# zypher-game/uzkge

Hardware: AMD Instinct MI355X
Metric: bn254_g1_msm_points_per_sec (higher is better)
Workload: dtype u256 (254-bit modular integers: 8 x u32 Montgomery limbs in HBM, 9 x 29-bit limbs in the two hot loops); 1 GPU; BN254 G1 MSM, 2^24 random points + uniform scalars per GPU, bases resident in HBM; points_per_gpu=16777216, total_points=16777216

## Files before the change

uzkge_amd/csrc/api.cpp:

```cpp
#include <algorithm>
#include <atomic>
#include <cstdarg>
#include <cstdlib>
#include <cstring>
#include <exception>
#include <new>

#include "anemoi29.hpp"
#include "ctx.hpp"
#include "fq12_29.hpp"
#include "g2_29.hpp"
#include "host_ec64.hpp"
#include "host_math.hpp"
#include "shufflecs_dev.hpp"
#include "matchcs_dev.hpp"

namespace uzk {

static thread_local char g_err[512] = "";

void set_error(const char* fmt, ...) {
    va_list ap;
    va_start(ap, fmt);
    vsnprintf(g_err, sizeof g_err, fmt, ap);
// ... 154 lines not shown
        device = c.want_device >= 0 ? c.want_device : s.device;
        UZK_TRY(device_cus_locked(s, device, &c.num_cus));
    }
    UZK_HIP(hipSetDevice(device));
    if (!c.ready) {
        UZK_HIP(hipStreamCreateWithFlags(&c.stream, hipStreamNonBlocking));
        c.device = device;
        c.ready = true;
    }
    return UZK_OK;
}

void devices_synchronize() {
    Shared& s = shared();
    std::vector<int> devs;
    {
        std::lock_guard<std::mutex> lk(s.mu);
        for (auto& kv : s.num_cus) devs.push_back(kv.first);
    }
    for (int d : devs) { (void)hipSetDevice(d); (void)hipDeviceSynchronize(); }
}

static void ctx_release(Ctx& c) {
    if (!c.ready) return;
    (void)hipSetDevice(c.device);
    (void)hipStreamSynchronize(c.stream);
    ntt_free_plans(c);
    g1ntt_free(c);
    srscheck_free(c);
    g2_free(c);
    g16_free(c);
    c.verify_ws.release();
    c.g16v_ws.release();
    c.ed_ws.release();
    c.shuffle_ws.release();
    c.match_ws.release();
    c.ed_gen.release();
    c.ed_gen_ready = false;
    c.pairing_ws.release();
    msm_free(c);
    poly_free(c);
    c.ntt_scratch[0].release(); c.ntt_scratch[1].release(); c.ntt_io.release(); c.msm_scalars.release();
    if (c.msm_tail_host) { (void)hipHostFree(c.msm_tail_host); c.msm_tail_host = nullptr; c.msm_tail_cap = 0; }
    for (auto& pe : c.prof_pending) { (void)hipEventDestroy(pe.e0); (void)hipEventDestroy(pe.e1); }
    c.prof_pending.clear();
    for (auto e : c.event_pool) (void)hipEventDestroy(e);
    c.event_pool.clear();
    (void)hipStreamDestroy(c.stream);
    c.stream = nullptr;
    c.cur_stream = nullptr;
    c.ready = false;
    c.device = -1;
}

static const Fp* as_fp(const uint64_t* p) { return reinterpret_cast<const Fp*>(p); }

static void copy_tuning(const Ctx& from, Ctx& to);
int ctx_init_internal(Ctx& c, int device) {
    c.want_device = device;
    {
        std::lock_guard<std::mutex> lk(default_ctx().mu);
        copy_tuning(default_ctx(), c);
    }
    CtxScope scope(&c);
    std::lock_guard<std::mutex> lk(c.mu);
    return require_ready();
}
void ctx_release_internal(Ctx& c) {
    std::lock_guard<std::mutex> lk(c.mu);
    ctx_release(c);
}

}

using namespace uzk;

#define API_LOCK std::lock_guard<std::mutex> _lk(ctx_mutex())

extern "C" {

#ifndef UZK_SRC_HASH
#define UZK_SRC_HASH "unstamped"
#endif
const char* uzk_version(void) { return "uzkge-amd 0.3 (gfx950) src:" UZK_SRC_HASH; }
const char* uzk_last_error(void) { return g_err; }

int uzk_device_count(void) try {
    int n = 0;
    if (hipGetDeviceCount(&n) != hipSuccess) return 0;
    return n;
} catch (...) { return uzk::on_exception("uzk_device_count"); }

int uzk_init(int device) try {
    API_LOCK;
    Shared& s = shared();
    {
        std::lock_guard<std::mutex> lk(s.mu);
        if (s.bound && s.device != device) {
            set_error("uzk_init(%d): already bound to device %d (one process per GPU)", device, s.device);
            return UZK_ERR_PARAMETER;
        }
        if (!s.bound) {
            int n = 0;
            if (hipGetDeviceCount(&n) != hipSuccess || n <= 0) {
                set_error("no HIP device visible: the MI355X backend has no CPU fallback");
                return UZK_ERR_DEVICE;
            }
            if (device < 0 || device >= n) {
                set_error("uzk_init(%d): %d device(s) visible", device, n);
                return UZK_ERR_PARAMETER;
            }
            UZK_TRY(bind_device_locked(s, device));
        }
    }
    return require_ready();
} catch (...) { return uzk::on_exception("uzk_init"); }

int uzk_shutdown(void) try {
    Shared& s = shared();
    coalesce_release_all();
    sharded_release_all();
    prover_release_all();
    vf_release_all();
    g2_release_all();
    g16_release_all();
    g16v_release_all();
    remark_release_all();
    std::lock_guard<std::mutex> lk(s.mu);
    if (!s.bound) return UZK_OK;
    ctx_release(default_ctx());
    for (auto& kv : s.contexts) { ctx_release(*kv.second); delete kv.second; }
    s.contexts.clear();
    s.epoch.fetch_add(1, std::memory_order_acq_rel);
    t_handle = 0;
    t_cached = nullptr;
    for (auto& kv : s.srs) {
        (void)hipSetDevice(kv.second.device);
        if (kv.second.owned && kv.second.d_points) (void)hipFree(kv.second.d_points);
        if (kv.second.d_table) (void)hipFree(kv.second.d_table);
    }
    s.srs.clear();
    s.num_cus.clear();
    s.bound = false;
    s.device = -1;
    return UZK_OK;
} catch (...) { return uzk::on_exception("uzk_shutdown"); }

namespace uzk {
static void copy_tuning(const Ctx& from, Ctx& to) {
    to.msm_window_bits = from.msm_window_bits;
    to.tune_no_precompute = from.tune_no_precompute; to.tune_ntt_tile = from.tune_ntt_tile; to.tune_ntt_two_pass = from.tune_ntt_two_pass; to.tune_small = from.tune_small;
    to.tune_chunk_log = from.tune_chunk_log; to.tune_verify_transcript = from.tune_verify_transcript; to.tune_stream_log = from.tune_stream_log; to.tune_stream_min_log = from.tune_stream_min_log;
    to.tune_seg_sort = from.tune_seg_sort; to.tune_arith29 = from.tune_arith29;
    to.tune_msm_taper = from.tune_msm_taper;
}
}
int uzk_ctx_create(uint64_t* ctx_out) try {
    if (!ctx_out) { set_error("uzk_ctx_create: null pointer"); return UZK_ERR_PARAMETER; }
    Ctx* c = new Ctx();
    {
        API_LOCK;
        int rc = require_ready();
        if (rc != UZK_OK) { delete c; return rc; }
        copy_tuning(ctx(), *c);
    }
    Shared& s = shared();
    std::lock_guard<std::mutex> lk(s.mu);
    const uint64_t h = s.next_ctx++;
    s.contexts[h] = c;
    *ctx_out = h;
    return UZK_OK;
} catch (...) { return uzk::on_exception("uzk_ctx_create"); }
int uzk_ctx_create_on(int device, uint64_t* ctx_out) try {
    if (!ctx_out) { set_error("uzk_ctx_create_on: null pointer"); return UZK_ERR_PARAMETER; }
    int n = 0;
    if (hipGetDeviceCount(&n) != hipSuccess || n <= 0) { set_error("no HIP device visible: the MI355X backend has no CPU fallback"); return UZK_ERR_DEVICE; }
    if (device < 0 || device >= n) { set_error("uzk_ctx_create_on(%d): %d device(s) visible", device, n); return UZK_ERR_PARAMETER; }
    Ctx* c = new Ctx();
    {
        API_LOCK;
        copy_tuning(ctx(), *c);
    }
    c->want_device = device;
    Shared& s = shared();
    std::lock_guard<std::mutex> lk(s.mu);
    const uint64_t h = s.next_ctx++;
    s.contexts[h] = c;
    *ctx_out = h;
    return UZK_OK;
} catch (...) { return uzk::on_exception("uzk_ctx_create_on"); }
int uzk_ctx_device(uint64_t handle, int* device_out) try {
    if (!device_out) { set_error("uzk_ctx_device: null pointer"); return UZK_ERR_PARAMETER; }
    Shared& s = shared();
    std::lock_guard<std::mutex> lk(s.mu);
    Ctx* c = nullptr;
    if (handle == 0) c = &default_ctx();
    else {
        auto it = s.contexts.find(handle);
        if (it == s.contexts.end()) { set_error("uzk_ctx_device: unknown context %llu", (unsigned long long)handle); return UZK_ERR_PARAMETER; }
        c = it->second;
    }
    *device_out = c->ready ? c->device : (c->want_device >= 0 ? c->want_device : (s.bound ? s.device : g_last_device));
    return UZK_OK;
} catch (...) { return uzk::on_exception("uzk_ctx_device"); }
int uzk_ctx_set_current(uint64_t handle) try {
    if (handle == 0) { t_handle = 0; t_cached = nullptr; return UZK_OK; }
    Shared& s = shared();
    std::lock_guard<std::mutex> lk(s.mu);
    auto it = s.contexts.find(handle);
    if (it == s.contexts.end()) { set_error("uzk_ctx_set_current: unknown context %llu", (unsigned long long)handle); return UZK_ERR_PARAMETER; }
    t_handle = handle;
    t_cached = it->second;
    t_epoch = s.epoch.load(std::memory_order_acquire);
    return UZK_OK;
} catch (...) { return uzk::on_exception("uzk_ctx_set_current"); }
int uzk_ctx_destroy(uint64_t handle) try {
    Shared& s = shared();
    Ctx* c = nullptr;
    {
        std::lock_guard<std::mutex> lk(s.mu);
        auto it = s.contexts.find(handle);
        if (it == s.contexts.end()) { set_error("uzk_ctx_destroy: unknown context %llu", (unsigned long long)handle); return UZK_ERR_PARAMETER; }
        c = it->second;
        s.contexts.erase(it);
        s.epoch.fetch_add(1, std::memory_order_acq_rel);
    }
    if (t_handle == handle) { t_handle = 0; t_cached = nullptr; }
    { std::lock_guard<std::mutex> lk(c->mu); ctx_release(*c); }
    delete c;
    return UZK_OK;
} catch (...) { return uzk::on_exception("uzk_ctx_destroy"); }

int uzk_ctx_current(uint64_t* ctx_out) try {
    if (!ctx_out) { set_error("uzk_ctx_current: null pointer"); return UZK_ERR_PARAMETER; }
    (void)ctx();
    *ctx_out = t_handle;
    return UZK_OK;
} catch (...) { return uzk::on_exception("uzk_ctx_current"); }
int uzk_ctx_wait(uint64_t other) try {
    Ctx* cur = &ctx();
    Ctx* oth = nullptr;
    if (other == 0) oth = &default_ctx();
    else {
        Shared& s = shared();
        std::lock_guard<std::mutex> lk(s.mu);
        auto it = s.contexts.find(other);
        if (it == s.contexts.end()) { set_error("uzk_ctx_wait: unknown context %llu", (unsigned long long)other); return UZK_ERR_PARAMETER; }
        oth = it->second;
    }
    if (oth == cur) return UZK_OK;
    std::unique_lock<std::mutex> l1(cur->mu, std::defer_lock), l2(oth->mu, std::defer_lock);
    std::lock(l1, l2);
    UZK_TRY(require_ready());
    if (!oth->ready) return UZK_OK;
    hipEvent_t ev = oth->get_event();
    struct Return { Ctx* c; hipEvent_t e; ~Return() { c->event_pool.push_back(e); } } back{oth, ev};
    UZK_HIP(hipEventRecord(ev, oth->stream));
    UZK_HIP(hipStreamWaitEvent(cur->stream, ev, 0));
    return UZK_OK;
} catch (...) { return uzk::on_exception("uzk_ctx_wait"); }

int uzk_dev_alloc(size_t bytes, void** d_out) try {
    API_LOCK;
    if (!d_out) { set_error("uzk_dev_alloc: null pointer"); return UZK_ERR_PARAMETER; }
    *d_out = nullptr;
    UZK_TRY(require_ready());
    if (bytes == 0) return UZK_OK;
    hipError_t e = hipMalloc(d_out, bytes);
    if (e != hipSuccess) {
        (void)hipGetLastError();
        *d_out = nullptr;
        set_error("uzk_dev_alloc(%zu): %s", bytes, hipGetErrorString(e));
        return UZK_ERR_DEVICE;
    }
    return UZK_OK;
} catch (...) { return uzk::on_exception("uzk_dev_alloc"); }
int uzk_dev_free(void* d_ptr) try {
    API_LOCK;
    if (!d_ptr) return UZK_OK;
    UZK_TRY(require_ready());
    UZK_HIP(hipStreamSynchronize(ctx().stream));
    UZK_HIP(hipFree(d_ptr));
    return UZK_OK;
} catch (...) { return uzk::on_exception("uzk_dev_free"); }
int uzk_host_alloc(size_t bytes, void** h_out) try {
    API_LOCK;
    if (!h_out) { set_error("uzk_host_alloc: null pointer"); return UZK_ERR_PARAMETER; }
    *h_out = nullptr;
    UZK_TRY(require_ready());
    if (bytes == 0) return UZK_OK;
    hipError_t e = hipHostMalloc(h_out, bytes, hipHostMallocDefault);
    if (e != hipSuccess) { (void)hipGetLastError(); *h_out = nullptr; set_error("uzk_host_alloc(%zu): %s", bytes, hipGetErrorString(e)); return UZK_ERR_DEVICE; }
    Shared& s = shared();
    std::lock_guard<std::mutex> lk(s.mu);
    s.pinned[*h_out] = bytes;
    return UZK_OK;
} catch (...) { return uzk::on_exception("uzk_host_alloc"); }
int uzk_host_free(void* h_ptr) try {
    API_LOCK;
    if (!h_ptr) return UZK_OK;
    UZK_TRY(require_ready());
    Shared& s = shared();
    size_t bytes = 0;
    {
        std::lock_guard<std::mutex> lk(s.mu);
        auto it = s.pinned.find(h_ptr);
        if (it == s.pinned.end()) { set_error("uzk_host_free: %p is not a block of uzk_host_alloc", h_ptr); return UZK_ERR_PARAMETER; }
// ... 1352 lines not shown
    API_LOCK;
    if (n > 0 && (!a || !b || !out)) { set_error("uzk_test_g2_kat: null pointer"); return UZK_ERR_PARAMETER; }
    if (op < 0 || (op > 5 && op < 10) || op > 14) { set_error("uzk_test_g2_kat: bad op"); return UZK_ERR_PARAMETER; }
    UZK_TRY(require_ready());
    return g2_op_device(ctx(), op, a, b, out, n);
} catch (...) { return uzk::on_exception("uzk_test_g2_kat"); }

int uzk_test_l29_kat(int field, int op, uint32_t param, const uint32_t* in, uint32_t* out, size_t n) try {
    API_LOCK;
    if (n > 0 && (!in || !out)) { set_error("uzk_test_l29_kat: null pointer"); return UZK_ERR_PARAMETER; }
    if (field < 0 || field > 1 || op < 0 || op > 22) { set_error("uzk_test_l29_kat: bad field/op"); return UZK_ERR_PARAMETER; }
    if (op == 20 && param > 5) { set_error("uzk_test_l29_kat: sub_off takes offsets 0 .. 5"); return UZK_ERR_PARAMETER; }
    if (op == 21 && !l29_sig_runnable(field, param)) { set_error("uzk_test_l29_kat: not a sub / to_wire / canon signature of this field"); return UZK_ERR_PARAMETER; }
    UZK_TRY(require_ready());
    return l29_op_device(ctx(), field, op, param, in, out, n);
} catch (...) { return uzk::on_exception("uzk_test_l29_kat"); }
int uzk_test_p29_kat(int op, const uint32_t* in, uint32_t* out, size_t n) try {
    API_LOCK;
    if (n > 0 && (!in || !out)) { set_error("uzk_test_p29_kat: null pointer"); return UZK_ERR_PARAMETER; }
    if (op < 0 || op > 3) { set_error("uzk_test_p29_kat: bad op"); return UZK_ERR_PARAMETER; }
    UZK_TRY(require_ready());
    return p29_op_device(ctx(), op, in, out, n);
} catch (...) { return uzk::on_exception("uzk_test_p29_kat"); }
int uzk_test_g2_raw_kat(int op, const uint32_t* in, uint32_t* out, size_t n) try {
    API_LOCK;
    if (n > 0 && (!in || !out)) { set_error("uzk_test_g2_raw_kat: null pointer"); return UZK_ERR_PARAMETER; }
    if (op < 0 || op > 4) { set_error("uzk_test_g2_raw_kat: bad op"); return UZK_ERR_PARAMETER; }
    UZK_TRY(require_ready());
    return g2_raw_op_device(ctx(), op, in, out, n);
} catch (...) { return uzk::on_exception("uzk_test_g2_raw_kat"); }
int uzk_test_fq12_raw_kat(int op, const uint32_t* in, uint32_t* out, size_t n) try {
    API_LOCK;
    if (n > (1u << 20) || (n > 0 && (!in || !out))) { set_error("uzk_test_fq12_raw_kat: null pointer or more than 2^20 elements"); return UZK_ERR_PARAMETER; }
    if (op < 0 || op > 12) { set_error("uzk_test_fq12_raw_kat: bad op"); return UZK_ERR_PARAMETER; }
    UZK_TRY(require_ready());
    return pairing_raw_kat_device(ctx(), op, in, out, (uint32_t)n);
} catch (...) { return uzk::on_exception("uzk_test_fq12_raw_kat"); }
int uzk_test_miller_step_raw(int op, const uint32_t* in, uint32_t* out, size_t n) try {
    API_LOCK;
    if (n > (1u << 20) || (n > 0 && (!in || !out))) { set_error("uzk_test_miller_step_raw: null pointer or more than 2^20 records"); return UZK_ERR_PARAMETER; }
    if (op < 0 || op > 1) { set_error("uzk_test_miller_step_raw: bad op"); return UZK_ERR_PARAMETER; }
    UZK_TRY(require_ready());
    return pairing_raw_step_device(ctx(), op, in, out, (uint32_t)n);
} catch (...) { return uzk::on_exception("uzk_test_miller_step_raw"); }
int uzk_test_ed_raw_kat(int op, const uint32_t* in, uint32_t* out, size_t n) try {
    API_LOCK;
    if (n > 0 && (!in || !out)) { set_error("uzk_test_ed_raw_kat: null pointer"); return UZK_ERR_PARAMETER; }
    if (op < 0 || op > 6) { set_error("uzk_test_ed_raw_kat: bad op"); return UZK_ERR_PARAMETER; }
    UZK_TRY(require_ready());
    return ed_raw_op_device(ctx(), op, in, out, n);
} catch (...) { return uzk::on_exception("uzk_test_ed_raw_kat"); }
int uzk_test_lanes(int op, const void* const* d_polys, const uint64_t* lane_strides, uint32_t count, const uint32_t* lens, const uint32_t* pts,
                   const uint64_t* args, uint32_t lanes, uint64_t len, uint64_t* out, int* kernel) try {
    API_LOCK;
    if (op < 0 || op > 1 || count == 0 || lanes == 0 || !kernel) { set_error("uzk_test_lanes: bad op / count / lanes"); return UZK_ERR_PARAMETER; }
    if (!d_polys || !lane_strides || !lens || !args || !out || (op == 1 && !pts)) { set_error("uzk_test_lanes: null pointer"); return UZK_ERR_PARAMETER; }
    for (uint32_t k = 0; k < count; ++k)
        if (!d_polys[k] || (op == 1 && pts[k] > 1)) { set_error("uzk_test_lanes: null polynomial or point index > 1"); return UZK_ERR_PARAMETER; }
    UZK_TRY(require_ready());
    return lanes_test(ctx(), op, d_polys, lane_strides, count, lens, pts, as_fp(args), lanes, len, reinterpret_cast<Fp*>(out), kernel);
} catch (...) { return uzk::on_exception("uzk_test_lanes"); }
int uzk_test_ntt_in_len(const void* d_in, uint64_t in_stride, void* d_out, uint64_t out_stride, uint64_t n, uint32_t batch,
                        const uint64_t* coset_shift_mont, uint64_t in_len) try {
    API_LOCK;
    if (!domain_supported(n)) {
        set_error("no evaluation domain of size %llu (need 2^k, k <= %d, or 3 * 2^k, k <= %d)", (unsigned long long)n, UZK_NTT_MAX_LOG2, UZK_NTT_MAX_LOG2_MIXED);
        return UZK_ERR_FFT;
    }
    if (!d_in || !d_out) { set_error("uzk_test_ntt_in_len: null pointer"); return UZK_ERR_PARAMETER; }
    UZK_TRY(require_ready());
    Ctx& c = ctx();
    UZK_TRY(ntt_run(c, static_cast<const Fp*>(d_in), static_cast<Fp*>(d_out), n, false,
                    coset_shift_mont ? as_fp(coset_shift_mont) : nullptr, batch, in_stride, out_stride, in_len));
    UZK_HIP(hipStreamSynchronize(c.stream));
    return UZK_OK;
} catch (...) { return uzk::on_exception("uzk_test_ntt_in_len"); }

int uzk_profile_enable(int on) try {
    API_LOCK;
    UZK_TRY(require_ready());
    Ctx& c = ctx();
    UZK_TRY(c.prof_collect());
    c.prof_on = on != 0;
    return UZK_OK;
} catch (...) { return uzk::on_exception("uzk_profile_enable"); }
int uzk_profile_reset(void) try {
    API_LOCK;
    Ctx& c = ctx();
    if (c.ready) UZK_TRY(c.prof_collect());
    c.prof_totals.clear();
    return UZK_OK;
} catch (...) { return uzk::on_exception("uzk_profile_reset"); }
int uzk_profile_get(const char* name, double* total_ms, uint64_t* launches) try {
    API_LOCK;
    Ctx& c = ctx();
    if (!name) { set_error("uzk_profile_get: null name"); return UZK_ERR_PARAMETER; }
    if (c.ready) UZK_TRY(c.prof_collect());
    auto it = c.prof_totals.find(name);
    if (total_ms) *total_ms = (it == c.prof_totals.end()) ? 0.0 : it->second.first;
    if (launches) *launches = (it == c.prof_totals.end()) ? 0 : it->second.second;
    return UZK_OK;
} catch (...) { return uzk::on_exception("uzk_profile_get"); }
int uzk_profile_dump(char* buf, size_t cap) try {
    API_LOCK;
    Ctx& c = ctx();
    if (!buf || cap == 0) { set_error("uzk_profile_dump: null buffer"); return UZK_ERR_PARAMETER; }
    if (c.ready) UZK_TRY(c.prof_collect());
    size_t off = 0;
    buf[0] = 0;
    for (auto& kv : c.prof_totals) {
        int w = snprintf(buf + off, cap - off, "%s %llu %.6f\n", kv.first.c_str(),
                         (unsigned long long)kv.second.second, kv.second.first);
        if (w < 0 || (size_t)w >= cap - off) break;
        off += (size_t)w;
    }
    return UZK_OK;
} catch (...) { return uzk::on_exception("uzk_profile_dump"); }
int uzk_sync(void) try {
    API_LOCK;
    UZK_TRY(require_ready());
    UZK_HIP(hipStreamSynchronize(ctx().stream));
    return UZK_OK;
} catch (...) { return uzk::on_exception("uzk_sync"); }
void* uzk_stream(void) {
    API_LOCK;
    if (require_ready() != UZK_OK) return nullptr;
    return ctx().stream;
}
int uzk_msm_set_window_bits(int c) try {
    API_LOCK;
    if (c != 0 && (c < 4 || c > 22)) { set_error("window bits must be 0 (auto) or 4..22"); return UZK_ERR_PARAMETER; }
    ctx().msm_window_bits = c;
    return UZK_OK;
} catch (...) { return uzk::on_exception("uzk_msm_set_window_bits"); }

int uzk_msm_plan_info(size_t n, int* window_bits, int* windows) try {
    API_LOCK;
    if (!window_bits || !windows || n == 0) { set_error("uzk_msm_plan_info: bad arguments"); return UZK_ERR_PARAMETER; }
    msm_plan_info(ctx(), n, window_bits, windows);
    return UZK_OK;
} catch (...) { return uzk::on_exception("uzk_msm_plan_info"); }

int uzk_tune(const char* key, int value) try {
    API_LOCK;
    if (!key) { set_error("uzk_tune: null key"); return UZK_ERR_PARAMETER; }
    Ctx& c = ctx();
    if (!std::strcmp(key, "msm_no_precompute")) c.tune_no_precompute = value;
    else if (!std::strcmp(key, "msm_stream_log")) c.tune_stream_log = (value >= -1 && value <= 26) ? value : 0;
    else if (!std::strcmp(key, "msm_stream_min_log")) c.tune_stream_min_log = (value >= 4 && value <= 26) ? value : 22;
    else if (!std::strcmp(key, "msm_chunk_log")) c.tune_chunk_log = (value >= 8 && value <= 26) ? value : 26;
    else if (!std::strcmp(key, "msm_small")) c.tune_small = value ? 1 : 0;
    else if (!std::strcmp(key, "msm_seg_sort")) c.tune_seg_sort = value;
    else if (!std::strcmp(key, "msm_taper")) c.tune_msm_taper = (value >= 0 && value <= 2) ? value : 1;
    else if (!std::strcmp(key, "ntt_tile")) c.tune_ntt_tile = (value == 1024 || value == 2048) ? value : 0;
    else if (!std::strcmp(key, "ntt_two_pass")) c.tune_ntt_two_pass = value ? 1 : 0;
    else if (!std::strcmp(key, "arith29")) c.tune_arith29 = value & 7;
    else if (!std::strcmp(key, "verify_transcript")) c.tune_verify_transcript = (value == 1 || value == 2) ? value : 0;
    else { set_error("uzk_tune: unknown key %s", key); return UZK_ERR_PARAMETER; }
    return UZK_OK;
} catch (...) { return uzk::on_exception("uzk_tune"); }

}
```

uzkge_amd/csrc/ctx.hpp:

```cpp
#pragma once
#include <hip/hip_runtime.h>

#include <cstdint>
#include <cstdlib>
#include <cstdio>
#include <chrono>
#include <map>
#include <mutex>
#include <string>
#include <vector>

#include "../../include/uzkge_gpu.h"
#include "../../include/uzkge_gpu_test.h"
#include "ec.hpp"

namespace uzk {

void set_error(const char* fmt, ...);
int on_exception(const char* fn) noexcept;

#define UZK_HIP(expr)                                                                      \
    do {                                                                                   \
        hipError_t _e = (expr);                                                            \
        if (_e != hipSuccess) {                                                            \
            (void)hipGetLastError();  \
            ::uzk::set_error("%s failed: %s (%s:%d)", #expr, hipGetErrorString(_e), __FILE__, __LINE__); \
            return UZK_ERR_DEVICE;                                                         \
        }                                                                                  \
    } while (0)

#define UZK_TRY(expr)                  \
    do {                               \
        int _rc = (expr);              \
        if (_rc != UZK_OK) return _rc; \
    } while (0)

struct DevBuf {
    void* p = nullptr;
    size_t cap = 0;
    int reserve(size_t bytes);
    void release();
    template <class T> T* as() const { return reinterpret_cast<T*>(p); }
};

struct ArgArena {
    char* h = nullptr;
    char* d = nullptr;
    size_t cap = 0, used = 0, uploaded = 0;
    int init(size_t bytes);
    void release();
    void reset() { used = 0; uploaded = 0; }
    template <class T> T* push(size_t count, const T** dev) {
        const size_t at = (used + 15) & ~(size_t)15, bytes = count * sizeof(T);
        if (at + bytes > cap) { *dev = nullptr; return nullptr; }
        used = at + bytes;
        *dev = reinterpret_cast<const T*>(d + at);
        return reinterpret_cast<T*>(h + at);
    }
    int upload(hipStream_t s);
};

struct ProfEntry {
    std::string name;
    hipEvent_t e0, e1;
};

struct NttPlan;
struct MsmWork;

struct Ctx {
    std::mutex mu;
    bool ready = false;
    int want_device = -1;
    int device = -1;
    hipStream_t stream = nullptr;
    hipStream_t stream2 = nullptr;
    hipStream_t cur_stream = nullptr;
    int num_cus = 256;
    bool prof_on = false;
    std::vector<ProfEntry> prof_pending;
    std::vector<hipEvent_t> event_pool;
    std::map<std::string, std::pair<double, uint64_t>> prof_totals;
    std::map<uint64_t, NttPlan*> ntt_plans;
    DevBuf ntt_scratch[2];
    DevBuf ntt_io;
    MsmWork* msm = nullptr;
    DevBuf msm_scalars;
    Fp* msm_tail_host = nullptr;
    size_t msm_tail_cap = 0;
    int msm_window_bits = 0;
    int tune_no_precompute = 0;
    int tune_ntt_two_pass = 1;
    int tune_ntt_tile = 0;
    int tune_small = 1;
    int tune_chunk_log = 26;
    int tune_stream_log = 0;
    int tune_stream_min_log = 22;
    int tune_arith29 = default_arith29();
    static int default_arith29() {
        static const int v = [] { const char* e = std::getenv("UZK_ARITH29"); return e ? std::atoi(e) : 7; }();
        return v;
    }
    int tune_seg_sort = 1;
    int tune_msm_taper = 1;
    DevBuf poly_tmp, poly_tmp2, poly_io, zpoly_tmp, open_tmp, poly_args;
    DevBuf poly_cnt;
    uint32_t trim_flip = 0;
    void* poly_host = nullptr;
    size_t poly_host_cap = 0;
    DevBuf ntt_sub;
    struct PowCache { Fp key; bool valid = false; uint64_t stamp = 0; DevBuf buf; };
    PowCache pow_cache[8];
    uint64_t pow_stamp = 0;
    std::vector<void*> ntt_fused;
    std::map<uint64_t, void*> g1ntt_plans;
    DevBuf g1ntt_work, g1ntt_prefix, g1ntt_io;
    DevBuf verify_ws;
    DevBuf srs_records, srs_weights, srs_points;
    void* g2 = nullptr;
    void* g16 = nullptr;
    DevBuf g16v_ws;
    DevBuf pairing_ws;
    std::vector<uint8_t> pairing_status;
    DevBuf ed_ws;
    DevBuf ed_gen;
    bool ed_gen_ready = false;
    DevBuf shuffle_ws;
    DevBuf match_ws;
    int tune_verify_transcript = 0;
    struct Srs {
        Affine* d_points = nullptr;
        size_t n = 0;
        bool owned = false;
        int device = 0;
        Affine* d_table = nullptr;
        int pre_c = 0;
        uint32_t pre_W = 0;
    };

    hipEvent_t get_event();
    void prof_begin(const char* name);
    void prof_end();
    int prof_collect();
};

struct ScalarView {
    const Fp* main = nullptr;
    uint64_t stride = 0;
    uint32_t n_main = 0;
    const Fp* tail = nullptr;
    uint32_t tail_n = 0;
    uint32_t group = 0xffffffffu;
    uint64_t group_stride = 0;
    static ScalarView dense(const Fp* p, size_t n) { ScalarView v; v.main = p; v.stride = n; v.n_main = (uint32_t)n; return v; }
    __host__ __device__ const Fp& at(uint32_t b, uint32_t i) const {
        return i < n_main ? main[(uint64_t)(b / group) * group_stride + (uint64_t)(b % group) * stride + i]
                          : tail[(uint64_t)b * tail_n + (i - n_main)];
    }
};

Ctx& ctx();
std::mutex& ctx_mutex();
int require_ready();
struct CtxScope {
    Ctx* prev;
    explicit CtxScope(Ctx* c);
    ~CtxScope();
    CtxScope(const CtxScope&) = delete;
    CtxScope& operator=(const CtxScope&) = delete;
};
int ctx_init_internal(Ctx& c, int device);
void ctx_release_internal(Ctx& c);
void devices_synchronize();
void coalesce_release_all();
void sharded_release_all();
uint64_t srs_insert(const Ctx::Srs& e);
bool srs_lookup(uint64_t handle, Ctx::Srs* out);
bool srs_erase(uint64_t handle, Ctx::Srs* out);
bool is_pinned_block(const void* p, size_t bytes);
int msm_dispatch_view(const Ctx::Srs& s, size_t offset, const ScalarView& sv, size_t n, uint32_t batch, Jac* out);
void prover_release_all();

struct HostScope {
    Ctx& c;
    const char* name;
    std::chrono::steady_clock::time_point t0;
    HostScope(Ctx& c_, const char* n) : c(c_), name(n), t0(std::chrono::steady_clock::now()) {}
    ~HostScope() {
        if (!c.prof_on) return;
        const double ms = std::chrono::duration<double, std::milli>(std::chrono::steady_clock::now() - t0).count();
        auto& e = c.prof_totals[name];
        e.first += ms; e.second += 1;
    }
};

struct KernelScope {
    Ctx& c;
    KernelScope(Ctx& c_, const char* name) : c(c_) { if (c.prof_on) c.prof_begin(name); }
    ~KernelScope() { if (c.prof_on) c.prof_end(); }
};

#define UZK_LAUNCH(c, name, kernel, grid, block, lds, stream, ...)                        \
    do {                                                                                   \
        {                                                                                  \
            ::uzk::KernelScope _ks((c), (name));                                           \
            hipLaunchKernelGGL(kernel, grid, block, lds, stream, __VA_ARGS__);             \
        }                                                                                  \
        UZK_HIP(hipGetLastError());                                                        \
    } while (0)

struct DeviceGuard {
    int prev = -1;
    explicit DeviceGuard(int device) {
        (void)hipGetDevice(&prev);
        (void)hipSetDevice(device);
    }
    ~DeviceGuard() { if (prev >= 0) (void)hipSetDevice(prev); }
    DeviceGuard(const DeviceGuard&) = delete;
    DeviceGuard& operator=(const DeviceGuard&) = delete;
};

int ntt_run(Ctx& c, const Fp* d_in, Fp* d_out, uint64_t n, bool inverse, const Fp* coset_shift_host, uint32_t batch,
            uint64_t in_stride = 0, uint64_t out_stride = 0, uint64_t in_len = 0);
void ntt_free_plans(Ctx& c);
int g1ntt_run(Ctx& c, const Affine* d_in, Affine* d_out, uint64_t n, bool inverse);
void g1ntt_op_count(uint64_t n, bool inverse, uint64_t* dbl_out, uint64_t* add_out);
void g1ntt_free(Ctx& c);
int vf_key_check(const uzk_vk_desc* d);
int vf_key_create(Ctx& c, const uzk_vk_desc* d, uint64_t* out);
bool vf_key_known(uint64_t h, uint32_t* cs_size, uint32_t* n_pi, uint32_t* proof_bytes, int* device);
int vf_key_release(uint64_t h);
void vf_release_all();
int vf_key_set_public_key(Ctx& c, uint64_t h, const Affine* pk);
int vf_fold_run(Ctx& c, uint64_t h, const uint8_t* proofs, const Fp* pi, uint32_t m, const Fp* weights, Jac* left_out, Jac* right_out,
                uint8_t* status_out, Fp* challenges_out);
int vf_keccak_test(Ctx& c, const uint8_t* msgs, const uint64_t* offsets, uint32_t count, uint8_t* out);
int srs_curve_run(Ctx& c, const Affine* d_points, uint64_t count, uzk_srs_curve_report* out);
int srs_weights_run(Ctx& c, const uint8_t seed[32], uint64_t first, uint64_t count, Fp* d_out);
void srs_weights_host(const uint8_t seed[32], uint64_t first, uint64_t count, Fp* out);
void srscheck_free(Ctx& c);
struct G2Affine;
struct G2Jac;
int g2_register(Ctx& c, const G2Affine* points, size_t n, uint64_t* handle_out);
bool g2_lookup(uint64_t handle, const G2Affine** d_points, size_t* n, int* device);
bool g2_release(uint64_t handle);
void g2_release_all();
void g2_free(Ctx& c);
int g2_msm_run(Ctx& c, const G2Affine* d_points, const Fp* d_scalars, size_t n, uint32_t batch, G2Jac* out_host);
void g2_fold_host(const G2Jac* partials, size_t count, G2Jac* out);
void g2_to_affine_host(const G2Jac* p, G2Affine* out);
int g2_op_device(Ctx& c, int op, const uint64_t* a, const uint64_t* b, uint64_t* out, size_t n);
int g2_raw_op_device(Ctx& c, int op, const uint32_t* in, uint32_t* out, size_t n);
int g16_key_check(const uzk_g16_key_desc* d, uint64_t* domain_out);
int g16_key_create(Ctx& c, const uzk_g16_key_desc* d, uint64_t* out);
bool g16_key_known(uint64_t h, uint32_t* n_vars, uint32_t* n_inputs, uint32_t* n_constraints, uint64_t* domain, int* device);
bool g16_key_release(uint64_t h);
void g16_release_all();
// ... 124 lines not shown
```

uzkge_amd/csrc/msm.hip:

```cpp
#include <algorithm>
#include <cmath>
#include <mutex>
#include <functional>
#include <memory>
#include <condition_variable>
#include <atomic>
#include <cstring>
#include <thread>
#include <vector>

#include "ctx.hpp"
#include "ec29.hpp"
#include "ecquad.hpp"
#include "ecquad29.hpp"
#include "ec29l.hpp"
#include "host_ec64.hpp"
#include "host_math.hpp"
#include "msm_cut.hpp"

namespace uzk {

constexpr uint32_t kSeg = 16;
constexpr uint32_t kSignBit = 0x80000000u;
constexpr uint32_t kCombineFan = 32;
// ... 48 lines not shown
        uint32_t out;
        if (d > half) { out = ((1u << c) - d) | kSignBit; carry = 1; }
        else { out = d; carry = 0; }
        if (out & ~kSignBit) out ^= flip;
        if (w >= w0) dst[(size_t)(w - w0) * n] = out;
    }
}

__global__ __launch_bounds__(1024) void msm_digits_hist_kernel(ScalarView scalars, uint32_t* __restrict__ digits,
                                                               uint32_t n, int c, int W, uint32_t shift, uint32_t bins,
                                                               uint32_t* __restrict__ counts) {
    extern __shared__ uint32_t hist[];
    const uint32_t ch = blockIdx.x, nch = gridDim.x, b = blockIdx.y;
    const uint32_t cs = (n + nch - 1) / nch;
    const uint32_t lo = min(n, ch * cs), hi = min(n, lo + cs);
    for (uint32_t k = threadIdx.x; k < (uint32_t)W * bins; k += blockDim.x) hist[k] = 0;
    __syncthreads();
    const uint32_t mask = (1u << c) - 1, half = 1u << (c - 1), bmask = bins - 1;
    for (uint32_t i = lo + threadIdx.x; i < hi; i += blockDim.x) {
        Fp k = Fr::from_mont(scalars.at(b, i));
        const uint32_t flip = msm_fold_scalar_sign(k);
        uint32_t carry = 0;
        uint32_t* dst = digits + (size_t)b * W * n + i;
        for (int w = 0; w < W; ++w) {
            uint32_t d = (k.v[0] & mask) + carry;
#pragma unroll
            for (int j = 0; j < 7; ++j) k.v[j] = __funnelshift_r(k.v[j], k.v[j + 1], c);
            k.v[7] >>= c;
            uint32_t out;
            if (d > half) { out = ((1u << c) - d) | kSignBit; carry = 1; }
            else { out = d; carry = 0; }
            if (out & ~kSignBit) out ^= flip;
            dst[(size_t)w * n] = out;
            const uint32_t mag = out & ~kSignBit;
            if (mag) atomicAdd(&hist[(uint32_t)w * bins + (((mag - 1) >> shift) & bmask)], 1u);
        }
    }
    __syncthreads();
    for (uint32_t k = threadIdx.x; k < (uint32_t)W * bins; k += blockDim.x) {
        const uint32_t w = k / bins, bin = k % bins;
        counts[(((size_t)b * W + w) * nch + ch) * bins + bin] = hist[k];
    }
}

struct RadixArgs {
    const uint32_t* digits;
    const uint2* in_entries;
    const uint32_t* seg_start;
    const uint32_t* seg_len;
    uint32_t n;
    uint32_t remap_cnt;
    uint32_t remap_stride, remap_off;
    const uint32_t* item_off;
    uint32_t nseg, chunk;
    uint32_t shift, mask, bins;
    uint32_t* counts;
    uint32_t* prefix;
    uint32_t* bin_base;
    uint32_t* bin_count;
    uint2* out_entries;
    uint32_t* out_vals;
    uint32_t pk_in_bits, pk_out_bits;
    uint32_t seg_min_len;
};
__device__ __forceinline__ uint32_t pk_key(uint32_t e, uint32_t idx_bits) { return e >> (idx_bits + 1); }
__device__ __forceinline__ uint32_t pk_val(uint32_t e, uint32_t idx_bits) {
    return (e & ((1u << idx_bits) - 1)) | (((e >> idx_bits) & 1u) << 31);
}
__device__ __forceinline__ uint32_t pk_make(uint32_t key_low, uint32_t val, uint32_t idx_bits) {
    return (key_low << (idx_bits + 1)) | ((val >> 31) << idx_bits) | (val & ~kSignBit);
}

template <bool FROM_DIGITS>
__device__ __forceinline__ bool radix_work(const RadixArgs& a, uint32_t item, uint32_t& seg, size_t& cidx, uint32_t& base,
                                           uint32_t& lo, uint32_t& hi) {
    if constexpr (FROM_DIGITS) {
        const uint32_t ch = blockIdx.x, nch = gridDim.x;
        seg = blockIdx.y;
        cidx = ((size_t)seg * nch + ch) * a.bins;
        base = 0;
        const uint32_t cs = (a.n + nch - 1) / nch;
        lo = min(a.n, ch * cs);
        hi = min(a.n, lo + cs);
        return true;
    } else {
        if (item >= a.item_off[a.nseg]) return false;
        uint32_t l = 0, h = a.nseg;
        while (h - l > 1) {
            const uint32_t mid = (l + h) >> 1;
            if (a.item_off[mid] <= item) l = mid; else h = mid;
        }
        seg = l;
        cidx = (size_t)item * a.bins;
        base = a.seg_start[seg];
        const uint32_t len = a.seg_len[seg];
        lo = min(len, (item - a.item_off[seg]) * a.chunk);
        hi = min(len, lo + a.chunk);
        return true;
    }
}
template <bool FROM_DIGITS, bool PK_IN>
__device__ __forceinline__ bool radix_load(const RadixArgs& a, uint32_t seg, uint32_t base, uint32_t k, uint32_t& key,
                                           uint32_t& val) {
    if constexpr (FROM_DIGITS) {
        const uint32_t d = a.digits[(size_t)seg * a.n + k];
        const uint32_t mag = d & ~kSignBit;
        key = mag - 1;
        uint32_t idx = k;
        if (a.remap_cnt) idx = (k / a.remap_cnt) * a.remap_stride + a.remap_off + (k % a.remap_cnt);
        val = idx | (d & kSignBit);
        return mag != 0;
    } else if constexpr (PK_IN) {
        const uint32_t e = reinterpret_cast<const uint32_t*>(a.in_entries)[(size_t)base + k];
        key = pk_key(e, a.pk_in_bits);
        val = pk_val(e, a.pk_in_bits);
        return true;
    } else {
        const uint2 e = a.in_entries[(size_t)base + k];
        key = e.x;
        val = e.y;
        return true;
    }
}

template <bool FROM_DIGITS, bool PK_IN>
__global__ __launch_bounds__(1024) void msm_radix_hist_kernel(RadixArgs a) {
    __shared__ uint32_t cnt[512];
    for (uint32_t item = blockIdx.x;; item += gridDim.x) {
        uint32_t seg, base, lo, hi;
        size_t cidx;
        if (!radix_work<FROM_DIGITS>(a, item, seg, cidx, base, lo, hi)) return;
        for (uint32_t b = threadIdx.x; b < a.bins; b += blockDim.x) cnt[b] = 0;
        __syncthreads();
        for (uint32_t k = lo + threadIdx.x; k < hi; k += blockDim.x) {
            if constexpr (FROM_DIGITS) {
                const uint32_t mag = a.digits[(size_t)seg * a.n + k] & ~kSignBit;
                if (mag) atomicAdd(&cnt[((mag - 1) >> a.shift) & a.mask], 1u);
            } else if constexpr (PK_IN) {
                const uint32_t e = reinterpret_cast<const uint32_t*>(a.in_entries)[(size_t)base + k];
                atomicAdd(&cnt[(pk_key(e, a.pk_in_bits) >> a.shift) & a.mask], 1u);
            } else {
                atomicAdd(&cnt[(a.in_entries[(size_t)base + k].x >> a.shift) & a.mask], 1u);
            }
        }
        __syncthreads();
        uint32_t* dst = a.counts + cidx;
        for (uint32_t b = threadIdx.x; b < a.bins; b += blockDim.x) dst[b] = cnt[b];
        if constexpr (FROM_DIGITS) return;
        __syncthreads();
    }
}

__global__ __launch_bounds__(512) void msm_radix_scan_kernel(RadixArgs a, uint32_t nch, const uint32_t* __restrict__ out_start_of,
                                                             uint32_t out_stride) {
    __shared__ uint32_t wsum[8];
    const uint32_t seg = blockIdx.x, b = threadIdx.x, G = gridDim.y, g = blockIdx.y;
    if (a.seg_min_len && a.seg_len[seg] <= a.seg_min_len) return;
    uint32_t run = 0;
    if (b < a.bins) {
        size_t first = (size_t)seg * nch;
        uint32_t cnt = nch;
        if (a.item_off) { first = a.item_off[seg]; cnt = a.item_off[seg + 1] - a.item_off[seg]; }
        const uint32_t per = (cnt + G - 1) / G;
        const uint32_t c0 = min(cnt, g * per), c1 = min(cnt, c0 + per);
        const uint32_t* p0 = a.counts + first * a.bins + b;
        uint32_t r0 = 0, r1 = 0, r2 = 0, r3 = 0;
        uint32_t ch = 0;
        for (; ch + 4 <= c0; ch += 4) {
            r0 += p0[(size_t)ch * a.bins];
            r1 += p0[(size_t)(ch + 1) * a.bins];
            r2 += p0[(size_t)(ch + 2) * a.bins];
            r3 += p0[(size_t)(ch + 3) * a.bins];
        }
        for (; ch < c0; ++ch) r0 += p0[(size_t)ch * a.bins];
        run = r0 + r1 + r2 + r3;
        for (ch = c0; ch < c1; ++ch) {
            const size_t at = (first + ch) * a.bins + b;
            const uint32_t v = a.counts[at];
            a.prefix[at] = run;
            run += v;
        }
    }
    if (g + 1 != G) return;
    uint32_t incl = run;
    for (int o = 1; o < 64; o <<= 1) {
        const uint32_t t = __shfl_up((int)incl, o);
        if ((int)(b & 63) >= o) incl += t;
    }
    if ((b & 63) == 63) wsum[b >> 6] = incl;
    __syncthreads();
    uint32_t pre = 0;
    for (uint32_t w = 0; w < (b >> 6); ++w) pre += wsum[w];
    const uint32_t excl = pre + incl - run;
    if (b < a.bins) {
        const uint32_t start = out_start_of ? out_start_of[seg] : seg * out_stride;
        a.bin_base[(size_t)seg * a.bins + b] = start + excl;
        a.bin_count[(size_t)seg * a.bins + b] = run;
    }
}

__global__ __launch_bounds__(1024) void msm_radix_items_kernel(const uint32_t* __restrict__ seg_len, uint32_t nseg,
                                                               uint32_t chunk, uint32_t* __restrict__ item_off, uint32_t min_len) {
    __shared__ uint32_t part[1024];
    const uint32_t tid = threadIdx.x;
    const uint32_t per = (nseg + 1023) / 1024;
    const uint32_t lo = min(nseg, tid * per), hi = min(nseg, lo + per);
    uint32_t s = 0;
    auto items_of = [&](uint32_t k) { const uint32_t l = seg_len[k]; return l > min_len ? (l + chunk - 1) / chunk : 0u; };
    for (uint32_t k = lo; k < hi; ++k) s += items_of(k);
    part[tid] = s;
    __syncthreads();
    for (uint32_t off = 1; off < 1024; off <<= 1) {
        uint32_t v = (tid >= off) ? part[tid - off] : 0;
        __syncthreads();
        part[tid] += v;
        __syncthreads();
    }
    uint32_t run = part[tid] - s;
    for (uint32_t k = lo; k < hi; ++k) { item_off[k] = run; run += items_of(k); }
    if (tid == 1023) item_off[nseg] = part[1023];
}

template <int TB, int E, bool FROM_DIGITS, bool OUT_VAL, bool PK_IN>
__global__ __launch_bounds__(TB) void msm_radix_scatter_kernel(RadixArgs a) {
    constexpr int TILE = TB * E;
    __shared__ uint2 buf[TILE];
    __shared__ uint32_t tcnt[512], toff[512], gcur[512], wsum[16];
    const uint32_t tid = threadIdx.x;
    for (uint32_t item = blockIdx.x;; item += gridDim.x) {
    uint32_t seg, base, lo, hi;
    size_t cidx;
    if (!radix_work<FROM_DIGITS>(a, item, seg, cidx, base, lo, hi)) return;
    const uint32_t* coff = a.prefix + cidx;
    for (uint32_t b = tid; b < a.bins; b += TB) gcur[b] = a.bin_base[(size_t)seg * a.bins + b] + coff[b];
    for (uint32_t t0 = lo; t0 < hi; t0 += TILE) {
        for (uint32_t b = tid; b < a.bins; b += TB) tcnt[b] = 0;
        __syncthreads();
        uint32_t key[E], val[E], rank[E];
        bool ok[E];
#pragma unroll
        for (int e = 0; e < E; ++e) {
            const uint32_t k = t0 + tid + e * TB;
            ok[e] = (k < hi) && radix_load<FROM_DIGITS, PK_IN>(a, seg, base, k, key[e], val[e]);
            if (ok[e]) rank[e] = atomicAdd(&tcnt[(key[e] >> a.shift) & a.mask], 1u);
        }
        __syncthreads();
        {
            const uint32_t ngroups = (a.bins + 63) / 64, lane = tid & 63;
            for (uint32_t g = tid >> 6; g < ngroups; g += TB / 64) {
                const uint32_t b = g * 64 + lane;
                const uint32_t v = (b < a.bins) ? tcnt[b] : 0;
                uint32_t incl = v;
                for (int o = 1; o < 64; o <<= 1) {
                    const uint32_t t = __shfl_up((int)incl, o);
                    if ((int)lane >= o) incl += t;
                }
                if (b < a.bins) toff[b] = incl - v;
                if (lane == 63) wsum[g] = incl;
            }
            __syncthreads();
            for (uint32_t b = tid; b < a.bins; b += TB) {
                uint32_t pre = 0;
                for (uint32_t g = 0; g < (b >> 6); ++g) pre += wsum[g];
                toff[b] += pre;
            }
            __syncthreads();
        }
#pragma unroll
        for (int e = 0; e < E; ++e) {
            if (ok[e]) buf[toff[(key[e] >> a.shift) & a.mask] + rank[e]] = make_uint2(key[e], val[e]);
        }
        __syncthreads();
        const uint32_t last = a.bins - 1;
        const uint32_t total = toff[last] + tcnt[last];
        for (uint32_t k = tid; k < total; k += TB) {
            const uint2 en = buf[k];
            const uint32_t bin = (en.x >> a.shift) & a.mask;
            const uint32_t pos = gcur[bin] + (k - toff[bin]);
            if constexpr (OUT_VAL) a.out_vals[pos] = en.y;
            else if (a.pk_out_bits)
                reinterpret_cast<uint32_t*>(a.out_entries)[pos] = pk_make(en.x & ((1u << a.shift) - 1), en.y, a.pk_out_bits);
            else a.out_entries[pos] = en;
        }
        __syncthreads();
        for (uint32_t b = tid; b < a.bins; b += TB) gcur[b] += tcnt[b];
        __syncthreads();
    }
    if constexpr (FROM_DIGITS) return;
    }
}

template <int TB, int E, int BUFN>
__global__ __launch_bounds__(TB, TB >= 512 ? 4 : 2) void msm_radix_segment_kernel(RadixArgs a) {
    constexpr uint32_t CAP = (uint32_t)TB * E;
    constexpr int MAXBINS = 512;
    __shared__ uint32_t buf[BUFN];
    __shared__ uint32_t cnt[MAXBINS], off[MAXBINS + 1], cur[MAXBINS], wsum[8];
    const uint32_t seg = blockIdx.x, tid = threadIdx.x;
    const uint32_t len = a.seg_len[seg];
    if (len > CAP) return;
    const uint32_t start = a.seg_start[seg];
    const uint32_t bins = a.bins;
    for (uint32_t b = tid; b < bins; b += TB) cnt[b] = 0;
    __syncthreads();
    const uint32_t* __restrict__ in = reinterpret_cast<const uint32_t*>(a.in_entries) + start;
    uint32_t e[E];
    const int mine = tid < len ? (int)((len - tid + TB - 1) / TB) : 0;
#pragma unroll
    for (int i = 0; i < E; ++i) e[i] = i < mine ? in[tid + (uint32_t)i * TB] : 0u;
#pragma unroll
    for (int i = 0; i < E; ++i)
        if (i < mine) atomicAdd(&cnt[(pk_key(e[i], a.pk_in_bits) >> a.shift) & a.mask], 1u);
    __syncthreads();
    {
        const uint32_t ngroups = (bins + 63) / 64, lane = tid & 63;
        for (uint32_t g = tid >> 6; g < ngroups; g += TB / 64) {
            const uint32_t b = g * 64 + lane;
            const uint32_t v = (b < bins) ? cnt[b] : 0;
            uint32_t incl = v;
            for (int o = 1; o < 64; o <<= 1) {
                const uint32_t t = __shfl_up((int)incl, o);
                if ((int)lane >= o) incl += t;
            }
            if (b < bins) off[b] = incl - v;
            if (lane == 63) wsum[g] = incl;
        }
        __syncthreads();
        for (uint32_t b = tid; b < bins; b += TB) {
            uint32_t pre = 0;
            for (uint32_t g = 0; g < (b >> 6); ++g) pre += wsum[g];
            const uint32_t o = off[b] + pre;
            off[b] = o;
            cur[b] = o;
            a.bin_base[(size_t)seg * bins + b] = start + o;
            a.bin_count[(size_t)seg * bins + b] = cnt[b];
        }
        if (tid == 0) off[bins] = len;
        __syncthreads();
    }
    uint32_t* __restrict__ out = a.out_vals + start;
    uint32_t b_lo = 0;
    while (b_lo < bins) {
        const uint32_t base = off[b_lo];
        uint32_t l = b_lo, h = bins + 1;
        while (h - l > 1) {
            const uint32_t mid = (l + h) >> 1;
            if (off[mid] - base <= (uint32_t)BUFN) l = mid; else h = mid;
        }
        const bool direct = (l == b_lo);
        const uint32_t b_hi = direct ? b_lo + 1 : l;
#pragma unroll
        for (int i = 0; i < E; ++i) {
            asm volatile("" : "+v"(e[i]));
            const uint32_t bin = (pk_key(e[i], a.pk_in_bits) >> a.shift) & a.mask;
            if (i < mine && bin >= b_lo && bin < b_hi) {
                const uint32_t pos = atomicAdd(&cur[bin], 1u);
                const uint32_t val = pk_val(e[i], a.pk_in_bits);
                if (direct) out[pos] = val; else buf[pos - base] = val;
            }
        }
        __syncthreads();
        if (!direct) {
            const uint32_t total = off[b_hi] - base;
            for (uint32_t k = tid; k < total; k += TB) out[base + k] = buf[k];
            __syncthreads();
        }
        b_lo = b_hi;
    }
}

template <int TB, int E, int BUFN>
__global__ __launch_bounds__(TB, 4) void msm_radix_chunk_kernel(RadixArgs a) {
    constexpr int MAXBINS = 512;
// ... 265 lines not shown
                                                               uint32_t* __restrict__ cursor, TaskDesc* __restrict__ desc) {
    const uint32_t n_big = *big_count, lane = threadIdx.x;
    for (uint32_t i = blockIdx.x; i < n_big; i += gridDim.x) {
        const BigBucket e = big[i];
        const uint32_t q = e.total / e.T, r = e.total - q * e.T;
        uint32_t p_hi = 0, p_lo = 0;
        if (lane == 0) {
            if (r) p_hi = atomicAdd(&cursor[min(q + 1, kLenBins - 1)], r);
            p_lo = atomicAdd(&cursor[min(q, kLenBins - 1)], e.T - r);
        }
        p_hi = (uint32_t)__shfl((int)p_hi, 0);
        p_lo = (uint32_t)__shfl((int)p_lo, 0);
        for (uint32_t j = lane; j < e.T; j += 64) {
            TaskDesc d;
            d.start = e.start + j * q + min(j, r);
            d.cnt = q + (j < r ? 1u : 0u);
            d.task = e.tid0 + j;
            d.pad = 0;
            desc[j < r ? p_hi + j : p_lo + (j - r)] = d;
        }
    }
}

__device__ __forceinline__ XYZZ& task_dst(XYZZ* __restrict__ partials, XYZZ* __restrict__ direct, uint32_t task) {
    return (task & kSignBit) ? direct[task & ~kSignBit] : partials[task];
}
__global__ __launch_bounds__(256, 4) void msm_accumulate29_kernel(const Affine* __restrict__ points,
                                                                  const uint32_t* __restrict__ sorted,
                                                                  const TaskDesc* __restrict__ desc,
                                                                  const uint32_t* __restrict__ win_base,
                                                                  XYZZ* __restrict__ partials, uint32_t W,
                                                                  uint32_t* __restrict__ exc_count,
                                                                  uint32_t* __restrict__ exc_list, XYZZ* __restrict__ direct = nullptr) {
#if defined(__HIP_DEVICE_COMPILE__)
    const uint32_t slot = blockIdx.x * blockDim.x + threadIdx.x;
    if (slot >= win_base[W]) return;
    const TaskDesc d = desc[slot];
    const uint32_t cnt = d.cnt;
    const uint32_t* run = sorted + d.start;
    Acc29 acc = acc29_inf();
    uint32_t e = run[0];
    Affine p = load_point(points, e & ~kSignBit);
    for (uint32_t k = 0; k < cnt; ++k) {
        const Affine cur = p;
        const bool neg = (e & kSignBit) != 0;
        if (k + 1 < cnt) {
            e = run[k + 1];
            p = load_point(points, e & ~kSignBit);
        }
        if (!acc29_madd(acc, cur, neg)) {
            exc_list[atomicAdd(exc_count, 1u)] = slot;
            return;
        }
    }
    task_dst(partials, direct, d.task) = acc29_to_xyzz(acc);
#endif
}
__global__ __launch_bounds__(256) void msm_accumulate_exc_kernel(const Affine* __restrict__ points,
                                                                 const uint32_t* __restrict__ sorted,
                                                                 const TaskDesc* __restrict__ desc,
                                                                 XYZZ* __restrict__ partials,
                                                                 const uint32_t* __restrict__ exc_count,
                                                                 const uint32_t* __restrict__ exc_list, XYZZ* __restrict__ direct = nullptr) {
    const uint32_t total = *exc_count;
    for (uint32_t i = blockIdx.x * blockDim.x + threadIdx.x; i < total; i += gridDim.x * blockDim.x) {
        const TaskDesc d = desc[exc_list[i]];
        const uint32_t* run = sorted + d.start;
        XYZZ acc = xyzz_inf();
        for (uint32_t k = 0; k < d.cnt; ++k) {
            const uint32_t e = run[k];
            xyzz_madd(acc, load_point(points, e & ~kSignBit), (e & kSignBit) != 0);
        }
        task_dst(partials, direct, d.task) = acc;
    }
}

__device__ __forceinline__ XYZZ xyzz_shfl_down(const XYZZ& p, int delta) {
    XYZZ r;
    const uint32_t* s = reinterpret_cast<const uint32_t*>(&p);
    uint32_t* d = reinterpret_cast<uint32_t*>(&r);
#pragma unroll
    for (int k = 0; k < 32; ++k) d[k] = (uint32_t)__shfl_down((int)s[k], delta);
    return r;
}
template <int GS>
__device__ __forceinline__ XYZZ fold_partials29(const XYZZ* __restrict__ src, uint32_t cnt, uint32_t sub) {
    P29 acc = p29_inf();
    for (uint32_t k = sub; k < cnt; k += GS) { const P29 q = p29_load(src[k]); p29_add(acc, q); }
    for (int o = GS / 2; o > 0; o >>= 1) {
        P29 q;
        const uint32_t* sp = reinterpret_cast<const uint32_t*>(&acc);
        uint32_t* dp = reinterpret_cast<uint32_t*>(&q);
#pragma unroll
        for (int w = 0; w < 36; ++w) dp[w] = (uint32_t)__shfl_down((int)sp[w], o);
        if (sub + (uint32_t)o < (uint32_t)GS) p29_add(acc, q);
    }
    return sub == 0 ? p29_store(acc) : xyzz_inf();
}
template <int GS>
__device__ __forceinline__ XYZZ fold_partials(const XYZZ* __restrict__ src, uint32_t cnt, uint32_t sub) {
    XYZZ acc = xyzz_inf();
    for (uint32_t k = sub; k < cnt; k += GS) { XYZZ q = src[k]; xyzz_add(acc, q); }
    for (int o = GS / 2; o > 0; o >>= 1) {
        XYZZ q = xyzz_shfl_down(acc, o);
        if (sub + (uint32_t)o < (uint32_t)GS) xyzz_add(acc, q);
    }
    return acc;
}

struct BigFold { uint32_t src, cnt, dst, pad; };
template <int GS>
__global__ __launch_bounds__(256) void msm_combine_kernel(const XYZZ* __restrict__ in, const uint32_t* __restrict__ in_cnt,
                                                          const uint32_t* __restrict__ in_off,
                                                          const uint32_t* __restrict__ in_base,
                                                          const uint32_t* __restrict__ task_off,
                                                          const uint32_t* __restrict__ win_base, XYZZ* __restrict__ out,
                                                          uint32_t NB, uint32_t W, uint32_t G, uint32_t* __restrict__ big_count,
                                                          BigFold* __restrict__ big, uint32_t big_thresh, int arith29) {
    const uint32_t gt = blockIdx.x * blockDim.x + threadIdx.x;
    const uint32_t tid = gt / GS, sub = gt % GS;
    if (tid >= win_base[W]) return;
    uint32_t w, b, j;
    find_task(tid, win_base, W, task_off, NB, w, b, j);
    const uint32_t total = in_cnt[(size_t)w * NB + b];
    const uint32_t first = j * G;
    const uint32_t cnt = min(G, total - first);
    const uint32_t at = in_base[w] + in_off[(size_t)w * NB + b] + first;
    if (GS == 1 && big != nullptr && cnt > big_thresh) {
        BigFold e; e.src = at; e.cnt = cnt; e.dst = tid; e.pad = 0;
        big[atomicAdd(big_count, 1u)] = e;
        return;
    }
    XYZZ acc = arith29 ? fold_partials29<GS>(in + at, cnt, sub) : fold_partials<GS>(in + at, cnt, sub);
    if (sub == 0) out[tid] = acc;
}
__global__ __launch_bounds__(64) void msm_fold_big_kernel(const XYZZ* __restrict__ in, const uint32_t* __restrict__ big_count,
                                                          const BigFold* __restrict__ big, XYZZ* __restrict__ out, int accumulate) {
    const uint32_t total = *big_count, lane = threadIdx.x;
    for (uint32_t i = blockIdx.x; i < total; i += gridDim.x) {
        const BigFold e = big[i];
        XYZZ acc = xyzz_inf();
        for (uint32_t k = lane; k < e.cnt; k += 64) { XYZZ q = in[e.src + k]; xyzz_add(acc, q); }
        for (int o = 32; o > 0; o >>= 1) {
            XYZZ q = xyzz_shfl_down(acc, o);
            if (lane + (uint32_t)o < 64) xyzz_add(acc, q);
        }
        if (lane == 0) {
            if (accumulate) { XYZZ prev = out[e.dst]; xyzz_add(prev, acc); out[e.dst] = prev; }
            else out[e.dst] = acc;
        }
    }
}

template <int GS>
__global__ __launch_bounds__(256) void msm_finalize_kernel(const XYZZ* __restrict__ in, const uint32_t* __restrict__ in_cnt,
                                                           const uint32_t* __restrict__ in_off,
                                                           const uint32_t* __restrict__ in_base,
                                                           XYZZ* __restrict__ buckets, uint32_t NB, uint32_t W, int accumulate,
                                                           uint32_t* __restrict__ big_count, BigFold* __restrict__ big, uint32_t big_thresh,
                                                           int skip_single, int arith29, MsmCut cut = MsmCut()) {
    const size_t gt = (size_t)blockIdx.x * blockDim.x + threadIdx.x;
    size_t t = gt / GS;
    const uint32_t sub = (uint32_t)(gt % GS);
    if (t >= (size_t)W * NB) return;
    if (GS == 1) t = (size_t)msm_cut_order(cut, W, t);
    const uint32_t w = (uint32_t)(t / NB);
    const uint32_t cnt = in_cnt[t];
    if (skip_single && cnt == 1) return;
    if (cut.n8 != 0) big_thresh = max(big_thresh, msm_cut_max_tasks(cut, w, (uint32_t)(t - (size_t)w * NB)));
    if (GS == 1 && big != nullptr && cnt > big_thresh) {
        BigFold e; e.src = in_base[w] + in_off[t]; e.cnt = cnt; e.dst = (uint32_t)t; e.pad = 0;
        big[atomicAdd(big_count, 1u)] = e;
        return;
    }
    XYZZ acc = arith29 ? fold_partials29<GS>(in + in_base[w] + in_off[t], cnt, sub) : fold_partials<GS>(in + in_base[w] + in_off[t], cnt, sub);
    if (sub == 0) {
        if (accumulate && cnt != 0) { XYZZ prev = buckets[t]; xyzz_add(prev, acc); buckets[t] = prev; }
        else if (!accumulate) buckets[t] = acc;
    }
}

__global__ __launch_bounds__(256) void msm_undirect_kernel(const XYZZ* __restrict__ buckets, const uint32_t* __restrict__ cnt,
                                                           const uint32_t* __restrict__ off, const uint32_t* __restrict__ base,
                                                           XYZZ* __restrict__ partials, uint32_t NB, uint64_t TBK) {
    const uint64_t t = (uint64_t)blockIdx.x * blockDim.x + threadIdx.x;
    if (t >= TBK || cnt[t] != 1) return;
    partials[base[t / NB] + off[t]] = buckets[t];
}

__global__ __launch_bounds__(256) void msm_reduce_kernel(const XYZZ* __restrict__ buckets, XYZZ* __restrict__ partials,
                                                         uint32_t nbk, uint32_t groups_per_window, uint32_t seg) {
    __shared__ XYZZ sh[256];
    const uint32_t w = blockIdx.y, tid = threadIdx.x;
    const uint32_t g = blockIdx.x * blockDim.x + tid;
    const XYZZ* bw = buckets + (size_t)w * nbk;
    XYZZ run = xyzz_inf(), acc = xyzz_inf();
    const uint64_t lo64 = (uint64_t)g * seg;
    if (lo64 < nbk) {
        const uint32_t lo = (uint32_t)lo64;
        const uint32_t hi = min(nbk, lo + seg);
        for (uint32_t idx = hi; idx-- > lo;) {
            XYZZ bk = bw[idx];
            xyzz_add(run, bk);
            xyzz_add(acc, run);
        }
        if (lo != 0 && !xyzz_is_inf(run)) {
            XYZZ m = xyzz_inf();
            for (int bit = 31 - __clz(lo); bit >= 0; --bit) {
                m = xyzz_dbl(m);
                if ((lo >> bit) & 1) xyzz_add(m, run);
            }
            xyzz_add(acc, m);
        }
    }
    sh[tid] = acc;
    __syncthreads();
    for (uint32_t s = 128; s > 0; s >>= 1) {
        if (tid < s) {
            XYZZ a = sh[tid];
            XYZZ b2 = sh[tid + s];
            xyzz_add(a, b2);
            sh[tid] = a;
        }
        __syncthreads();
    }
    if (tid == 0) partials[(size_t)w * groups_per_window + blockIdx.x] = sh[0];
}
__global__ __launch_bounds__(256) void msm_fold_partials_kernel(const XYZZ* __restrict__ partials, XYZZ* __restrict__ out,
                                                                uint32_t groups) {
    __shared__ XYZZ sh[256];
    const uint32_t w = blockIdx.x, tid = threadIdx.x;
    XYZZ acc = xyzz_inf();
    for (uint32_t g = tid; g < groups; g += 256) { XYZZ q = partials[(size_t)w * groups + g]; xyzz_add(acc, q); }
    sh[tid] = acc;
    __syncthreads();
    for (uint32_t s = 128; s > 0; s >>= 1) {
        if (tid < s) {
            XYZZ a = sh[tid];
            XYZZ b2 = sh[tid + s];
            xyzz_add(a, b2);
            sh[tid] = a;
        }
        __syncthreads();
    }
    if (tid == 0) out[w] = sh[0];
}

__device__ __forceinline__ void wg_suffix_scan(XYZZ* sh, uint32_t tid, XYZZ& mine, uint32_t width) {
    sh[tid] = mine;
    __syncthreads();
    for (uint32_t off = 1; off < width; off <<= 1) {
        XYZZ v = (tid + off < 256) ? sh[tid + off] : xyzz_inf();
        __syncthreads();
        xyzz_add(mine, v);
        sh[tid] = mine;
        __syncthreads();
    }
}
__device__ __forceinline__ void wg_tree_sum(XYZZ* sh, uint32_t tid, const XYZZ& mine, uint32_t width) {
    sh[tid] = mine;
    __syncthreads();
    for (uint32_t s = width >> 1; s > 0; s >>= 1) {
        if (tid < s) {
            XYZZ a = sh[tid];
            XYZZ b2 = sh[tid + s];
            xyzz_add(a, b2);
            sh[tid] = a;
        }
        __syncthreads();
    }
}
__global__ __launch_bounds__(256) void msm_reduce_scan_kernel(const XYZZ* __restrict__ buckets, XYZZ* __restrict__ part_p1,
                                                              XYZZ* __restrict__ part_r, uint32_t nbk,
                                                              uint32_t groups_per_window, uint32_t seg, uint32_t log_seg) {
    __shared__ XYZZ sh[256];
    const uint32_t w = blockIdx.y, tid = threadIdx.x;
    const uint32_t g = blockIdx.x * blockDim.x + tid;
    const XYZZ* bw = buckets + (size_t)w * nbk;
    XYZZ run = xyzz_inf(), acc = xyzz_inf();
    const uint64_t lo64 = (uint64_t)g * seg;
    if (lo64 < nbk) {
        const uint32_t lo = (uint32_t)lo64;
        const uint32_t hi = min(nbk, lo + seg);
        for (uint32_t idx = hi; idx-- > lo;) {
            XYZZ bk = bw[idx];
            xyzz_add(run, bk);
            xyzz_add(acc, run);
        }
    }
    const uint64_t lanes_w = ((uint64_t)nbk + seg - 1) / seg;
    const uint64_t mine_first = (uint64_t)blockIdx.x * 256;
    uint32_t active = lanes_w > mine_first ? (uint32_t)min((uint64_t)256, lanes_w - mine_first) : 1u;
    uint32_t width = 1;
    while (width < active) width <<= 1;
    XYZZ suf = run;
    wg_suffix_scan(sh, tid, suf, width);
    XYZZ above = (tid + 1 < 256) ? sh[tid + 1] : xyzz_inf();
    const XYZZ total = sh[0];
    __syncthreads();
    for (uint32_t d = 0; d < log_seg; ++d) above = xyzz_dbl(above);
    xyzz_add(acc, above);
    wg_tree_sum(sh, tid, acc, width);
    if (tid == 0) {
        part_p1[(size_t)w * groups_per_window + blockIdx.x] = sh[0];
        part_r[(size_t)w * groups_per_window + blockIdx.x] = total;
    }
}
__global__ __launch_bounds__(256) void msm_fold_scan_kernel(const XYZZ* __restrict__ part_p1, const XYZZ* __restrict__ part_r,
                                                            XYZZ* __restrict__ out, uint32_t groups, uint32_t log_shift) {
    __shared__ XYZZ sh[256];
    const uint32_t w = blockIdx.x, tid = threadIdx.x;
    XYZZ r = tid < groups ? part_r[(size_t)w * groups + tid] : xyzz_inf();
    XYZZ p1 = tid < groups ? part_p1[(size_t)w * groups + tid] : xyzz_inf();
    uint32_t width = 1;
    while (width < groups) width <<= 1;
    if (groups > 1) {
        wg_suffix_scan(sh, tid, r, width);
        XYZZ above = (tid + 1 < 256) ? sh[tid + 1] : xyzz_inf();
        __syncthreads();
        if (!xyzz_is_inf(above)) {
            for (uint32_t d = 0; d < log_shift; ++d) above = xyzz_dbl(above);
            xyzz_add(p1, above);
        }
    }
    wg_tree_sum(sh, tid, p1, width);
    if (tid == 0) out[w] = sh[0];
}

__global__ __launch_bounds__(256, 3) void msm_class_sums_kernel(const XYZZ* __restrict__ buckets, XYZZ* __restrict__ out, uint32_t nbk,
                                                              uint32_t log_s, uint32_t nb2, int arith29) {
    __shared__ XYZZ sh[256];
    const uint32_t tile = blockIdx.x, w = blockIdx.y, cols = blockIdx.z, t = threadIdx.x;
    const uint32_t Lc = 1u << log_s, H = nbk >> log_s;
    const XYZZ* bw = buckets + (size_t)w * nbk;
    XYZZ* ow = out + ((size_t)w * 2 + cols) * nb2;
    const uint32_t G = cols ? H / 8 : Lc / 8;
    const XYZZ* src = cols ? bw + (tile * (256 / G) + t / G) : bw + (size_t)tile * 2048 + (size_t)t * 8;
    const size_t step = cols ? Lc : 1, first = cols ? (size_t)(t % G) * 8 * Lc : 0;
    if (arith29) {
        P29 acc = p29_inf();
#pragma unroll 1
        for (uint32_t k = 0; k < 8; ++k) { const P29 q = p29_load(src[first + k * step]); p29_add(acc, q); }
        sh[t] = p29_store(acc);
    } else {
        XYZZ acc = xyzz_inf();
#pragma unroll 1
        for (uint32_t k = 0; k < 8; ++k) { XYZZ q = src[first + k * step]; xyzz_add(acc, q); }
        sh[t] = acc;
    }
    __syncthreads();
    uint32_t live = 256;
    const uint32_t qi = t >> 2, ql = t & 3;
    for (uint32_t g = G; g > 1;) {
        const uint32_t f = (g % 4 == 0) ? 4 : 2;
        live /= f;
        XYZZ a;
        if (live <= 64) {
            if (qi < live) {
                a = sh[qi * f];
                for (uint32_t k = 1; k < f; ++k) { const XYZZ q = sh[qi * f + k]; xyzz_add_quad(a, q, ql); }
            }
            __syncthreads();
            if (qi < live && ql == 0) sh[qi] = a;
        } else {
            if (t < live) {
                a = sh[t * f];
                for (uint32_t k = 1; k < f; ++k) { XYZZ q = sh[t * f + k]; xyzz_add(a, q); }
            }
            __syncthreads();
            if (t < live) sh[t] = a;
        }
        __syncthreads();
        g /= f;
    }
    if (t < 256 / G) {
        const uint32_t cls = tile * (256 / G) + t;
        if (!cols) { if (cls != 0) ow[cls - 1] = sh[t]; }
        else ow[cls] = sh[t];
    }
    if (tile == 0) for (uint32_t k = (cols ? Lc : H - 1) + t; k < nb2; k += 256) ow[k] = xyzz_inf();
}

constexpr uint32_t kQuadLanes = 64, kLogQuadLanes = 6;
__device__ __forceinline__ void wgq_suffix_scan(XYZZ* sh, uint32_t t, uint32_t q, XYZZ& mine, uint32_t width) {
    if (q == 0) sh[t] = mine;
    __syncthreads();
    for (uint32_t off = 1; off < width; off <<= 1) {
        const bool has = t + off < kQuadLanes;
        XYZZ v;
        if (has) v = sh[t + off];
        __syncthreads();
        if (has) { xyzz_add_quad(mine, v, q); if (q == 0) sh[t] = mine; }
        __syncthreads();
    }
}
__device__ __forceinline__ void wgq_tree_sum(XYZZ* sh, uint32_t t, uint32_t q, XYZZ mine, uint32_t width) {
    if (q == 0) sh[t] = mine;
    __syncthreads();
    for (uint32_t s = width >> 1; s > 0; s >>= 1) {
        if (t < s) {
            const XYZZ v = sh[t + s];
            xyzz_add_quad(mine, v, q);
            if (q == 0) sh[t] = mine;
        }
        __syncthreads();
    }
}
__global__ __launch_bounds__(kQuadLanes * 4) void msm_reduce_scan_quad_kernel(const XYZZ* __restrict__ buckets, XYZZ* __restrict__ part_p1,
                                                                    XYZZ* __restrict__ part_r, uint32_t nbk,
                                                                    uint32_t groups_per_window, uint32_t seg, uint32_t log_seg) {
    __shared__ XYZZ sh[kQuadLanes];
    const uint32_t w = blockIdx.y, t = threadIdx.x >> 2, q = threadIdx.x & 3;
    const uint32_t g = blockIdx.x * kQuadLanes + t;
    const XYZZ* bw = buckets + (size_t)w * nbk;
    XYZZ run = xyzz_inf(), acc = xyzz_inf();
    const uint64_t lo64 = (uint64_t)g * seg;
    if (lo64 < nbk) {
        const uint32_t lo = (uint32_t)lo64;
        const uint32_t hi = min(nbk, lo + seg);
        for (uint32_t idx = hi; idx-- > lo;) {
            const XYZZ bk = bw[idx];
            xyzz_add_quad(run, bk, q);
            xyzz_add_quad(acc, run, q);
        }
    }
    const uint64_t lanes_w = ((uint64_t)nbk + seg - 1) / seg;
    const uint64_t mine_first = (uint64_t)blockIdx.x * kQuadLanes;
    const uint32_t active = lanes_w > mine_first ? (uint32_t)min((uint64_t)kQuadLanes, lanes_w - mine_first) : 1u;
    uint32_t width = 1;
    while (width < active) width <<= 1;
    XYZZ suf = run;
    wgq_suffix_scan(sh, t, q, suf, width);
    XYZZ above = (t + 1 < kQuadLanes) ? sh[t + 1] : xyzz_inf();
    const XYZZ total = sh[0];
    __syncthreads();
    for (uint32_t d = 0; d < log_seg; ++d) xyzz_dbl_quad(above, q);
    xyzz_add_quad(acc, above, q);
    wgq_tree_sum(sh, t, q, acc, width);
    if (threadIdx.x == 0) {
        part_p1[(size_t)w * groups_per_window + blockIdx.x] = sh[0];
        part_r[(size_t)w * groups_per_window + blockIdx.x] = total;
    }
}
__global__ __launch_bounds__(kQuadLanes * 4) void msm_fold_scan_quad_kernel(const XYZZ* __restrict__ part_p1, const XYZZ* __restrict__ part_r,
                                                                  XYZZ* __restrict__ out, uint32_t groups, uint32_t log_shift) {
    __shared__ XYZZ sh[kQuadLanes];
    const uint32_t w = blockIdx.x, t = threadIdx.x >> 2, q = threadIdx.x & 3;
    XYZZ r = t < groups ? part_r[(size_t)w * groups + t] : xyzz_inf();
    XYZZ p1 = t < groups ? part_p1[(size_t)w * groups + t] : xyzz_inf();
    uint32_t width = 1;
    while (width < groups) width <<= 1;
    if (groups > 1) {
        wgq_suffix_scan(sh, t, q, r, width);
        XYZZ above = (t + 1 < kQuadLanes) ? sh[t + 1] : xyzz_inf();
        __syncthreads();
        if (!xyzz_is_inf(above)) {
            for (uint32_t d = 0; d < log_shift; ++d) xyzz_dbl_quad(above, q);
            xyzz_add_quad(p1, above, q);
        }
    }
    wgq_tree_sum(sh, t, q, p1, width);
    if (threadIdx.x == 0) out[w] = sh[0];
}

struct SmallChunk { uint32_t first, cnt; };
constexpr uint32_t kSmallFan = 16;
constexpr int kSmallMaxLevels = 4;
constexpr uint32_t kSmallNone = 0xFFFFFFFFu;
struct SmallLevels {
    uint32_t nl;
    uint32_t pbase[kSmallMaxLevels + 1];
    uint32_t dbase[kSmallMaxLevels + 1];
};

__device__ __forceinline__ uint32_t block_excl_scan_u32(uint32_t v, uint32_t* wsum, uint32_t tid, uint32_t nthreads,
                                                       uint32_t& total) {
    const uint32_t lane = tid & 63;
    uint32_t incl = v;
    for (int o = 1; o < 64; o <<= 1) {
        const uint32_t t = (uint32_t)__shfl_up((int)incl, o);
        if ((int)lane >= o) incl += t;
    }
    __syncthreads();
    if (lane == 63) wsum[tid >> 6] = incl;
    __syncthreads();
    uint32_t pre = 0, tot = 0;
    for (uint32_t w = 0; w < nthreads / 64; ++w) {
        const uint32_t x = wsum[w];
        if (w < (tid >> 6)) pre += x;
        tot += x;
    }
    total = tot;
    return pre + incl - v;
}
__device__ __forceinline__ uint32_t small_find(const uint32_t* off, uint32_t nb, uint32_t t) {
    uint32_t lo = 0, hi = nb;
    while (hi - lo > 1) {
        const uint32_t mid = (lo + hi) >> 1;
        if (off[mid] <= t) lo = mid; else hi = mid;
    }
    return lo;
}

__global__ __launch_bounds__(1024) void msm_small_sort_kernel(const uint32_t* __restrict__ digits, uint32_t n, uint32_t NBL,
                                                              uint32_t L, uint32_t* __restrict__ sorted,
                                                              TaskDesc* __restrict__ desc, SmallChunk* __restrict__ cdesc,
                                                              uint32_t* __restrict__ bucket_ref, uint2* __restrict__ slot_chunks,
                                                              uint32_t* __restrict__ counters, SmallLevels lv, uint32_t W,
                                                              uint32_t pre_stride, uint32_t pre_off) {
    extern __shared__ uint32_t sm_small[];
    uint32_t* cnt = sm_small;
    uint32_t* start = cnt + NBL;
    uint32_t* toff = start + NBL + 1;
    uint32_t* coff = toff + NBL + 1;
    uint32_t* cur = coff + NBL + 1;
    uint32_t* misc = cur + NBL;
    uint32_t* wsum = misc + 4;
    uint32_t* stage = wsum + 17;
    const uint32_t slot = blockIdx.x, tid = threadIdx.x;
    const uint32_t* dg = digits + (size_t)slot * n;
    for (uint32_t b = tid; b < NBL; b += 1024) { cnt[b] = 0; cur[b] = 0; }
    __syncthreads();
    for (uint32_t i = tid; i < n; i += 1024) {
        const uint32_t mag = dg[i] & ~kSignBit;
        if (mag) atomicAdd(&cnt[mag - 1], 1u);
    }
    __syncthreads();
    const uint32_t e = tid < NBL ? cnt[tid] : 0u;
    const uint32_t tk = (e + L - 1) / L;
    uint32_t tot_e, tot_t;
    const uint32_t es = block_excl_scan_u32(e, wsum, tid, 1024, tot_e);
    const uint32_t ts = block_excl_scan_u32(tk, wsum, tid, 1024, tot_t);
    if (tid < NBL) { start[tid] = es; toff[tid] = ts; }
    if (tid == 0) {
        start[NBL] = tot_e; toff[NBL] = tot_t;
        misc[0] = atomicAdd(&counters[0], tot_t);
    }
    __syncthreads();
    const uint32_t tbase = misc[0];
    const uint32_t idx_base = pre_stride ? (slot % W) * pre_stride + pre_off : 0u;
    for (uint32_t i = tid; i < n; i += 1024) {
        const uint32_t d = dg[i], mag = d & ~kSignBit;
        if (mag) stage[start[mag - 1] + atomicAdd(&cur[mag - 1], 1u)] = (idx_base + i) | (d & kSignBit);
    }
    __syncthreads();
    uint32_t* so = sorted + (size_t)slot * n;
    for (uint32_t k = tid; k < tot_e; k += 1024) so[k] = stage[k];
    for (uint32_t t = tid; t < tot_t; t += 1024) {
        const uint32_t b = small_find(toff, NBL, t), j = t - toff[b];
        const uint32_t total = cnt[b], T = toff[b + 1] - toff[b];
        const uint32_t q = total / T, r = total - q * T;
        TaskDesc d;
        d.start = slot * n + start[b] + j * q + min(j, r);
        d.cnt = q + (j < r ? 1u : 0u);
        d.task = tbase + t;
        d.pad = 0;
        desc[tbase + t] = d;
    }
    uint32_t have = tk, first = tbase + ts;
    for (uint32_t lvl = 1; lvl <= lv.nl; ++lvl) {
        const uint32_t ck = have > 1 ? (have + kSmallFan - 1) / kSmallFan : 0u;
        uint32_t tot_c;
        const uint32_t cs = block_excl_scan_u32(ck, wsum, tid, 1024, tot_c);
        if (tid < NBL) { coff[tid] = cs; cnt[tid] = have; cur[tid] = first; }
        if (tid == 0) {
            coff[NBL] = tot_c;
            misc[1] = atomicAdd(&counters[lvl], tot_c);
            slot_chunks[(size_t)slot * kSmallMaxLevels + (lvl - 1)] = make_uint2(misc[1], tot_c);
        }
        __syncthreads();
        const uint32_t cbase = misc[1];
        for (uint32_t ch = tid; ch < tot_c; ch += 1024) {
            const uint32_t b = small_find(coff, NBL, ch), j = ch - coff[b];
            SmallChunk cd;
            cd.first = cur[b] + j * kSmallFan;
            cd.cnt = min(kSmallFan, cnt[b] - j * kSmallFan);
            cdesc[lv.dbase[lvl] + cbase + ch] = cd;
        }
        if (ck) { have = ck; first = lv.pbase[lvl] + cbase + cs; }
    }
    if (tid < NBL) bucket_ref[(size_t)slot * NBL + tid] = have ? first : kSmallNone;
}

template <bool QUAD, int GS>
__global__ __launch_bounds__(256) void msm_small_fold_kernel(XYZZ* __restrict__ P, const SmallChunk* __restrict__ cdesc,
                                                             const uint32_t* __restrict__ count, uint32_t out_base, int arith29) {
    constexpr uint32_t LPL = QUAD ? 4 : 1;
    const uint32_t gt = blockIdx.x * blockDim.x + threadIdx.x;
    const uint32_t group = gt / (LPL * GS), sub = (gt / LPL) % GS, q = gt & 3;
    if (group >= *count) return;
    const SmallChunk cd = cdesc[group];
    if constexpr (QUAD) {
        if (arith29) {
            P29 acc = p29_inf();
            for (uint32_t k = sub; k < cd.cnt; k += GS) { const P29 v = p29_load(P[cd.first + k]); p29_add_quad(acc, v, q); }
#pragma unroll
            for (int o = GS / 2; o > 0; o >>= 1) {
                P29 v;
                const uint32_t* sp = reinterpret_cast<const uint32_t*>(&acc);
// ... 211 lines not shown
    return acc;
}
constexpr int kPreRun = 16;
__global__ __launch_bounds__(64) void msm_precompute_kernel(const Affine* __restrict__ prev, Affine* __restrict__ out,
                                                            Fp* __restrict__ tmp_z, Fp* __restrict__ tmp_p, uint32_t n,
                                                            int c) {
    const uint32_t t = blockIdx.x * blockDim.x + threadIdx.x;
    const uint32_t lo = t * kPreRun;
    if (lo >= n) return;
    const uint32_t hi = min(n, lo + kPreRun);
    Fp prod = Fq::one();
    for (uint32_t i = lo; i < hi; ++i) {
        XYZZ a = xyzz_from_affine(prev[i]);
        for (int d = 0; d < c; ++d) a = xyzz_dbl(a);
        Affine xy;
        Fp z;
        if (xyzz_is_inf(a)) {
            xy.x = Fq::zero(); xy.y = Fq::zero(); z = Fq::one();
        } else {
            xy.x = Fq::mul(a.x, a.zz);
            xy.y = Fq::mul(a.y, a.zzz);
            z = a.zz;
        }
        out[i] = xy;
        tmp_z[i] = z;
        tmp_p[i] = prod;
        prod = Fq::mul(prod, z);
    }
    Fp inv = fq_inv_pow(prod);
    for (uint32_t i = hi; i-- > lo;) {
        Fp zi = Fq::mul(inv, tmp_p[i]);
        inv = Fq::mul(inv, tmp_z[i]);
        Fp zi2 = Fq::sqr(zi);
        Affine xy = out[i];
        xy.x = Fq::mul(xy.x, zi2);
        xy.y = Fq::mul(xy.y, Fq::mul(zi2, zi));
        out[i] = xy;
    }
}

__global__ __launch_bounds__(64) void msm_precompute_column_kernel(Affine* __restrict__ table, Fp* __restrict__ tmp_z,
                                                                   Fp* __restrict__ tmp_p, uint32_t n, int c, uint32_t W) {
    const uint32_t i = blockIdx.x * blockDim.x + threadIdx.x;
    if (i >= n) return;
    XYZZ a = xyzz_from_affine(table[i]);
    Fp prod = Fq::one();
    for (uint32_t j = 1; j < W; ++j) {
        for (int d = 0; d < c; ++d) a = xyzz_dbl(a);
        Affine xy;
        Fp z;
        if (xyzz_is_inf(a)) { xy.x = Fq::zero(); xy.y = Fq::zero(); z = Fq::one(); }
        else { xy.x = Fq::mul(a.x, a.zz); xy.y = Fq::mul(a.y, a.zzz); z = a.zz; }
        const size_t at = (size_t)j * n + i;
        table[at] = xy;
        tmp_z[at] = z;
        tmp_p[at] = prod;
        prod = Fq::mul(prod, z);
    }
    Fp inv = fq_inv_pow(prod);
    for (uint32_t j = W - 1; j >= 1; --j) {
        const size_t at = (size_t)j * n + i;
        const Fp zi = Fq::mul(inv, tmp_p[at]);
        inv = Fq::mul(inv, tmp_z[at]);
        const Fp zi2 = Fq::sqr(zi);
        Affine xy = table[at];
        xy.x = Fq::mul(xy.x, zi2);
        xy.y = Fq::mul(xy.y, Fq::mul(zi2, zi));
        table[at] = xy;
    }
}

static int choose_window_bits(size_t n, int forced) {
    if (forced >= 4 && forced <= 22) return forced;
    int lg = 0;
    while ((1ull << (lg + 1)) <= n) ++lg;
    if (lg <= 16) return 8;
    if (lg <= 18) return 15;
    if (lg <= 20) return 16;
    return 17;
}
int msm_precompute_window_bits(size_t n, int forced) {
    if (forced >= 4 && forced <= 24) return forced;
    if (n <= (1u << 15)) return n <= 256 ? 5 : n <= 2048 ? 7 : 8;
    int lg = 0;
    while ((1ull << (lg + 1)) <= n) ++lg;
    return std::max(8, std::min(22, lg - 2));
}

void msm_free(Ctx& c) {
    if (!c.msm) return;
    for (int q = 0; q < 2; ++q) {
        MsmWork* m = &c.msm[q];
        m->digits.release(); m->bucket_count.release(); m->bucket_start.release(); m->sorted.release();
        m->buckets.release(); m->partials.release(); m->win_sums.release(); m->class_sums.release(); m->big.release(); m->small.release(); m->task_desc.release(); m->exc.release();
        for (int k = 0; k < 2; ++k) {
            m->ent[k].release(); m->lvl_cnt[k].release(); m->lvl_off[k].release(); m->lvl_part[k].release();
        }
        for (int k = 0; k < kMaxPasses; ++k) {
            m->counts[k].release(); m->segs_start[k].release(); m->segs_len[k].release(); m->items[k].release();
        }
        if (m->h_sums) (void)hipHostFree(m->h_sums);
        if (m->h_max) (void)hipHostFree(m->h_max);
    }
    delete[] c.msm;
    c.msm = nullptr;
    if (c.stream2) { (void)hipStreamDestroy(c.stream2); c.stream2 = nullptr; }
}

int msm_build_table(Ctx& c, const Affine* d_points, size_t n, int cb, Affine** table_out, uint32_t* W_out) {
    const uint32_t W = (uint32_t)msm_num_windows(cb);
    if ((uint64_t)W * n >= (1ull << 31)) {
        set_error("precompute: W*n = %llu exceeds 2^31 - 1", (unsigned long long)W * n);
        return UZK_ERR_PARAMETER;
    }
    Affine* table = nullptr;
    UZK_HIP(hipMalloc(reinterpret_cast<void**>(&table), (size_t)W * n * sizeof(Affine)));
    Fp *tz = nullptr, *tp = nullptr;
    hipError_t e = hipMalloc(reinterpret_cast<void**>(&tz), n * sizeof(Fp));
    if (e == hipSuccess) e = hipMalloc(reinterpret_cast<void**>(&tp), n * sizeof(Fp));
    if (e == hipSuccess) e = hipMemcpyAsync(table, d_points, n * sizeof(Affine), hipMemcpyDeviceToDevice, c.stream);
    if (e == hipSuccess && n <= (1u << 16) && W > 1) {
        (void)hipFree(tz); (void)hipFree(tp); tz = tp = nullptr;
        e = hipMalloc(reinterpret_cast<void**>(&tz), (size_t)W * n * sizeof(Fp));
        if (e == hipSuccess) e = hipMalloc(reinterpret_cast<void**>(&tp), (size_t)W * n * sizeof(Fp));
        if (e == hipSuccess) {
            KernelScope ks(c, "msm_precompute");
            hipLaunchKernelGGL(msm_precompute_column_kernel, dim3((unsigned)((n + 63) / 64)), dim3(64), 0, c.stream, table, tz, tp,
                               (uint32_t)n, cb, W);
        }
        if (e == hipSuccess) e = hipGetLastError();
        if (e == hipSuccess) e = hipStreamSynchronize(c.stream);
    } else if (e == hipSuccess) {
        const uint32_t threads = (uint32_t)((n + kPreRun - 1) / kPreRun);
        for (uint32_t j = 1; j < W; ++j) {
            KernelScope ks(c, "msm_precompute");
            hipLaunchKernelGGL(msm_precompute_kernel, dim3((threads + 63) / 64), dim3(64), 0, c.stream,
                               table + (size_t)(j - 1) * n, table + (size_t)j * n, tz, tp, (uint32_t)n, cb);
        }
        e = hipGetLastError();
        if (e == hipSuccess) e = hipStreamSynchronize(c.stream);
    }
    if (tz) (void)hipFree(tz);
    if (tp) (void)hipFree(tp);
    if (e != hipSuccess) {
        (void)hipFree(table);
        set_error("precompute failed: %s", hipGetErrorString(e));
        return UZK_ERR_DEVICE;
    }
    *table_out = table;
    *W_out = W;
    return UZK_OK;
}

struct SortPass { uint32_t shift, bins, nseg, nch, chunk, items_bound; };
constexpr int kSegCfgs = 6;
constexpr uint32_t kSegCap[kSegCfgs] = {128 * 12, 256 * 12, 256 * 24, 256 * 40, 512 * 40, 512 * 72};

struct MsmGroup {
    MsmWork* m = nullptr;
    hipStream_t st = nullptr;
    bool pre = false;
    int cb = 0;
    uint32_t W_total = 0, w0 = 0, W = 0, n32 = 0, batch = 0;
    uint64_t per_poly = 0, entries = 0, TBK = 0, bound0 = 0, part_cap = 0;
    uint32_t kb = 0, NBL = 0, S0 = 0, seg_n = 0, NB = 0, Wd = 0, RW = 0, seg = 0, groups = 0, L = 0;
    int P = 0;
    bool scan_reduce = false, quad_reduce = false;
    bool direct = false;
    uint32_t class_s = 0, nb2 = 0;
    uint32_t rl = 256;
    uint32_t pk_bits = 0;
    MsmCut cut;
    SortPass sp[kMaxPasses];
    uint32_t *cnt_cur = nullptr, *off_cur = nullptr, *base_cur = nullptr;
    XYZZ* part_cur = nullptr;
};

static int msm_group_plan(Ctx& c, MsmGroup& g, size_t n, uint32_t batch, int cb, bool pre, uint32_t W_total, uint32_t w0,
                          uint32_t W, uint64_t idx_span = 0) {
    g.pre = pre; g.cb = cb; g.W_total = W_total; g.w0 = w0; g.W = W; g.n32 = (uint32_t)n; g.batch = batch;
    g.per_poly = (uint64_t)W * n;
    g.entries = g.per_poly * batch;
    if (g.entries >= (1ull << 31)) { set_error("msm: batch*W*n overflows the 31-bit index space"); return UZK_ERR_PARAMETER; }
    g.kb = (uint32_t)cb - 1;
    g.NBL = 1u << g.kb;
    g.S0 = pre ? batch : batch * W;
    g.seg_n = pre ? (uint32_t)g.per_poly : g.n32;
    g.NB = std::min<uint32_t>(g.NBL, 1u << 15);
    while (((uint64_t)g.S0 * g.NBL) / g.NB > 1024 && g.NB < (1u << 15)) g.NB <<= 1;
    g.Wd = (uint32_t)(((uint64_t)g.S0 * g.NBL) / g.NB);
    g.TBK = (uint64_t)g.Wd * g.NB;
    if (g.Wd > 1024) { set_error("msm: too many bucket windows (%u): lower the batch", g.Wd); return UZK_ERR_PARAMETER; }
    g.RW = pre ? batch : batch * W;
    const uint64_t total_buckets = (uint64_t)g.RW * g.NBL;
    g.quad_reduce = total_buckets <= (1u << 19);
    g.scan_reduce = g.quad_reduce || g.NBL <= (1u << 14);
    if (g.scan_reduce) {
        uint32_t sg = 8u;
        if (g.quad_reduce) {
            sg = 1;
            while ((uint64_t)sg * 32768 < total_buckets) sg <<= 1;
        }
        while (sg & (sg - 1)) sg &= sg - 1;
        g.rl = g.quad_reduce ? kQuadLanes : 256u;
        if (g.quad_reduce && g.NBL <= 4 * g.rl) sg = std::max<uint32_t>(sg, g.NBL / g.rl);
        sg = std::max<uint32_t>(1, std::min<uint32_t>(sg, g.NBL / g.rl));
        while ((g.NBL + sg * g.rl - 1) / (sg * g.rl) > g.rl) sg <<= 1;
        g.seg = sg;
    } else {
        g.seg = std::max<uint32_t>(1, std::min<uint32_t>(kSeg, g.NBL / 256));
    }
    g.groups = (g.NBL + g.seg * g.rl - 1) / (g.seg * g.rl);
    g.class_s = 0; g.nb2 = 0;
    if (g.NBL >= 4096 && g.NBL <= (1u << 18) && (uint64_t)g.RW * 2 <= 65535) {
        g.class_s = 8;
        g.nb2 = std::max<uint32_t>(256, g.NBL >> 8);
    }
    const uint64_t all_entries = (uint64_t)W_total * n * batch;
    const uint64_t mean_pop = (pre ? (uint64_t)W_total * n : (uint64_t)n) >> g.kb;
    g.L = (uint32_t)std::max<uint64_t>(16, std::min<uint64_t>(256, std::min<uint64_t>(4 * mean_pop, all_entries / 200000)));
    g.cut = msm_cut_plan(g.L, g.NB, g.entries, c.tune_msm_taper);
    g.bound0 = msm_task_bound(g.cut, g.Wd, g.entries);
    g.part_cap = g.bound0 + 2 * g.TBK;
    g.P = g.kb <= 9 ? 1 : (g.kb <= 18 ? 2 : 3);
    g.pk_bits = 0;
    if (g.P == 2 && (!pre || idx_span)) {
        uint32_t ib = 1;
        while ((1ull << ib) < (pre ? idx_span : (uint64_t)g.seg_n)) ++ib;
        const uint32_t first_bits = std::min<uint32_t>(9, g.kb - 1);
        if (ib + 1 + (g.kb - first_bits) <= 32) g.pk_bits = ib;
    }
    uint32_t rem = g.kb, nseg = g.S0;
    for (int p = 0; p < g.P; ++p) {
        uint32_t bits = (rem + (uint32_t)(g.P - p) - 1) / (uint32_t)(g.P - p);
        if (g.pk_bits && p == 0) bits = std::min<uint32_t>(9, g.kb - 1);
        rem -= bits;
        g.sp[p].shift = rem;
        g.sp[p].bins = 1u << bits;
        g.sp[p].nseg = nseg;
        const uint64_t avg = std::max<uint64_t>(1, (g.S0 * (uint64_t)g.seg_n) / nseg);
        g.sp[p].nch = (uint32_t)std::max<uint64_t>(1, std::min<uint64_t>(1024, avg / 32768));
        if (p == 0 && g.pk_bits && avg <= (1ull << 25)) g.sp[p].nch = (uint32_t)((avg + 32767) / 32768);
        g.sp[p].chunk = (p == g.P - 1) ? 16384u : 32768u;
        g.sp[p].items_bound = (uint32_t)(g.entries / g.sp[p].chunk) + nseg;
        nseg *= g.sp[p].bins;
    }
    MsmWork& m = *g.m;
    UZK_TRY(m.digits.reserve((size_t)g.entries * 4));
    UZK_TRY(m.sorted.reserve((size_t)g.entries * 4));
    UZK_TRY(m.bucket_count.reserve((size_t)g.TBK * 4));
    UZK_TRY(m.bucket_start.reserve((size_t)g.TBK * 4));
    UZK_TRY(m.buckets.reserve((size_t)g.TBK * sizeof(XYZZ)));
    UZK_TRY(m.partials.reserve((size_t)2 * g.RW * std::max<uint32_t>(g.groups, g.class_s ? 2 * (g.nb2 / 256 + 1) : 0) * sizeof(XYZZ)));
    UZK_TRY(m.win_sums.reserve((size_t)g.RW * 2 * sizeof(XYZZ)));
    if (g.class_s) UZK_TRY(m.class_sums.reserve((size_t)g.RW * 2 * g.nb2 * sizeof(XYZZ)));
    for (int p = 0; p < g.P; ++p) {
        UZK_TRY(m.counts[p].reserve((size_t)(p == 0 ? 2 * g.sp[p].nseg * g.sp[p].nch : g.sp[p].items_bound) * g.sp[p].bins * 4));
        if (p > 0) UZK_TRY(m.items[p].reserve(((size_t)g.sp[p].nseg + 1) * 4));
        if (p + 1 < g.P) {
            UZK_TRY(m.segs_start[p].reserve((size_t)g.sp[p].nseg * g.sp[p].bins * 4));
            UZK_TRY(m.segs_len[p].reserve((size_t)g.sp[p].nseg * g.sp[p].bins * 4));
            UZK_TRY(m.ent[p & 1].reserve((size_t)g.entries * sizeof(uint2)));
        }
    }
    for (int k = 0; k < 2; ++k) {
        UZK_TRY(m.lvl_cnt[k].reserve((size_t)g.TBK * 4));
        UZK_TRY(m.lvl_off[k].reserve((size_t)g.TBK * 4));
    }
    UZK_TRY(m.lvl_part[0].reserve((size_t)g.part_cap * sizeof(XYZZ)));
    UZK_TRY(m.small.reserve(16384));
    UZK_TRY(m.task_desc.reserve((size_t)g.bound0 * sizeof(TaskDesc)));
    UZK_TRY(m.exc.reserve((size_t)g.bound0 * 4));
    if (m.h_sums_cap < (size_t)g.RW * 2) {
        if (m.h_sums) (void)hipHostFree(m.h_sums);
        UZK_HIP(hipHostMalloc(reinterpret_cast<void**>(&m.h_sums), (size_t)g.RW * 2 * sizeof(XYZZ), hipHostMallocDefault));
        m.h_sums_cap = (size_t)g.RW * 2;
    }
    if (!m.h_max) UZK_HIP(hipHostMalloc(reinterpret_cast<void**>(&m.h_max), 64, hipHostMallocDefault));
    return UZK_OK;
}

static int msm_group_phase1(Ctx& c, MsmGroup& g, const Affine* points, const ScalarView& d_scalars, uint32_t pre_stride,
                            uint32_t pre_off, bool direct_ok = true) {
    MsmWork& m = *g.m;
    hipStream_t st = g.st;
    c.cur_stream = st;
    uint32_t* digits = m.digits.as<uint32_t>();
    uint32_t* sorted = m.sorted.as<uint32_t>();
    uint32_t* bcount = m.bucket_count.as<uint32_t>();
    uint32_t* bstart = m.bucket_start.as<uint32_t>();
    uint32_t* sm = m.small.as<uint32_t>();
    uint32_t* win_tot = sm;
    uint32_t* d_max = sm + 3200;
    UZK_HIP(hipMemsetAsync(d_max, 0, (3912 - 3200) * 4, st));
    const bool fused_hist = !g.pre && g.w0 == 0 && g.W == g.W_total && g.sp[0].nch >= 256 &&
                            (size_t)g.W * g.sp[0].bins * 4 <= 64 * 1024;
    if (fused_hist) {
        KernelScope ks(c, "msm_digits");
        hipLaunchKernelGGL(msm_digits_hist_kernel, dim3(g.sp[0].nch, g.batch), dim3(1024), (size_t)g.W * g.sp[0].bins * 4, st,
                           d_scalars, digits, g.n32, g.cb, (int)g.W, g.sp[0].shift, g.sp[0].bins, m.counts[0].as<uint32_t>());
    } else {
        KernelScope ks(c, "msm_digits");
        const uint64_t tot = (uint64_t)g.n32 * g.batch;
        hipLaunchKernelGGL(msm_digits_kernel, dim3((unsigned)((tot + 255) / 256)), dim3(256), 0, st, d_scalars, digits, g.n32,
                           g.batch, g.cb, (int)g.W_total, (int)g.w0, (int)g.W, (uint32_t*)nullptr);
    }
    for (int p = 0; p < g.P; ++p) {
        const bool first = (p == 0), last = (p == g.P - 1);
        const SortPass& sp = g.sp[p];
        RadixArgs a{};
        a.shift = sp.shift; a.bins = sp.bins; a.mask = sp.bins - 1;
        a.counts = m.counts[p].as<uint32_t>();
        a.prefix = first ? a.counts + (size_t)sp.nseg * sp.nch * sp.bins : a.counts;
        if (first) {
            a.digits = digits;
            a.n = g.seg_n;
            if (g.pre) { a.remap_cnt = g.n32; a.remap_stride = pre_stride; a.remap_off = pre_off; }
        } else {
            a.in_entries = m.ent[(p - 1) & 1].as<uint2>();
            a.seg_start = m.segs_start[p - 1].as<uint32_t>();
            a.seg_len = m.segs_len[p - 1].as<uint32_t>();
        }
        if (g.pk_bits) { if (first) a.pk_out_bits = g.pk_bits; else a.pk_in_bits = g.pk_bits; }
        if (last) { a.bin_base = bstart; a.bin_count = bcount; a.out_vals = sorted; }
        else {
            a.bin_base = m.segs_start[p].as<uint32_t>(); a.bin_count = m.segs_len[p].as<uint32_t>();
            a.out_entries = m.ent[p & 1].as<uint2>();
        }
        int seg_cfg = -1;
        if (last && !first && g.P == 2 && a.pk_in_bits && c.tune_seg_sort && sp.bins <= 512) {
            const double mean = (double)g.seg_n / (double)g.sp[0].bins;
            const double need = mean + 8.0 * std::sqrt(mean) + 64.0;
            for (int k = 0; k < kSegCfgs; ++k)
                if ((double)kSegCap[k] >= need) { seg_cfg = k; break; }
            if (c.tune_seg_sort >= 10) seg_cfg = std::min(kSegCfgs - 1, c.tune_seg_sort - 10);
            if (seg_cfg >= 0) a.seg_min_len = kSegCap[seg_cfg];
        }
        if (!first) {
            a.item_off = m.items[p].as<uint32_t>();
            a.nseg = sp.nseg;
            a.chunk = sp.chunk;
            KernelScope ks(c, "msm_sort_items");
            hipLaunchKernelGGL(msm_radix_items_kernel, dim3(1), dim3(1024), 0, st, a.seg_len, a.nseg, a.chunk,
                               m.items[p].as<uint32_t>(), a.seg_min_len);
        }
        const dim3 grid = first ? dim3(sp.nch, sp.nseg) : dim3(seg_cfg >= 0 ? std::min<uint32_t>(sp.items_bound, 2048u) : sp.items_bound);
        {
            const size_t wgs = first ? 2 * (size_t)grid.x * grid.y : (size_t)sp.items_bound;
            const size_t ent_bytes = g.pk_bits ? 4 : sizeof(uint2);
            const bool ok = m.counts[p].cap >= wgs * sp.bins * 4 &&
                            (last ? (m.bucket_start.cap >= (size_t)sp.nseg * sp.bins * 4 && m.bucket_count.cap >= (size_t)sp.nseg * sp.bins * 4 &&
                                     m.sorted.cap >= (size_t)g.entries * 4)
                                  : (m.segs_start[p].cap >= (size_t)sp.nseg * sp.bins * 4 && m.segs_len[p].cap >= (size_t)sp.nseg * sp.bins * 4 &&
                                     m.ent[p & 1].cap >= (size_t)g.entries * ent_bytes)) &&
                            (first || m.items[p].cap >= ((size_t)sp.nseg + 1) * 4);
            if (!ok) { set_error("msm: sort pass %d: a workspace is smaller than its launch needs (internal error)", p); return UZK_ERR_DEVICE; }
        }
        if (seg_cfg >= 0) {
            KernelScope ks(c, "msm_sort_segment");
            const dim3 sgrid(sp.nseg);
            switch (seg_cfg) {
                case 0: hipLaunchKernelGGL((msm_radix_segment_kernel<128, 12, 1536>), sgrid, dim3(128), 0, st, a); break;
                case 1: hipLaunchKernelGGL((msm_radix_segment_kernel<256, 12, 3072>), sgrid, dim3(256), 0, st, a); break;
                case 2: hipLaunchKernelGGL((msm_radix_segment_kernel<256, 24, 6144>), sgrid, dim3(256), 0, st, a); break;
                case 3: hipLaunchKernelGGL((msm_radix_segment_kernel<256, 40, 10240>), sgrid, dim3(256), 0, st, a); break;
                case 4: hipLaunchKernelGGL((msm_radix_segment_kernel<512, 40, 18432>), sgrid, dim3(512), 0, st, a); break;
                default: hipLaunchKernelGGL((msm_radix_segment_kernel<512, 72, 18432>), sgrid, dim3(512), 0, st, a); break;
            }
        }
        if (!(first && fused_hist)) {
            KernelScope ks(c, "msm_sort_hist");
            if (first) hipLaunchKernelGGL((msm_radix_hist_kernel<true, false>), grid, dim3(1024), 0, st, a);
            else if (a.pk_in_bits) hipLaunchKernelGGL((msm_radix_hist_kernel<false, true>), grid, dim3(256), 0, st, a);
            else hipLaunchKernelGGL((msm_radix_hist_kernel<false, false>), grid, dim3(256), 0, st, a);
        }
        {
            KernelScope ks(c, "msm_sort_scan");
            const uint32_t scan_g = first ? std::max<uint32_t>(1, std::min<uint32_t>(sp.nch / 16, 1024 / std::max<uint32_t>(1, sp.nseg))) : 1u;
            hipLaunchKernelGGL(msm_radix_scan_kernel, dim3(sp.nseg, scan_g), dim3(512), 0, st, a, sp.nch,
                               first ? (const uint32_t*)nullptr : a.seg_start, first ? g.seg_n : 0u);
        }
        {
            KernelScope ks(c, "msm_sort_scatter");
            const uint32_t cs0 = first ? (g.seg_n + sp.nch - 1) / sp.nch : 0u;
            if (first && !last && a.pk_out_bits && sp.bins <= 512 && cs0 <= 32768 && !g.pre)
                hipLaunchKernelGGL((msm_radix_chunk_kernel<512, 64, 18176>), grid, dim3(512), 0, st, a);
            else if (first && last) hipLaunchKernelGGL((msm_radix_scatter_kernel<1024, 8, true, true, false>), grid, dim3(1024), 0, st, a);
            else if (first && g.entries >= (1ull << 26))
                hipLaunchKernelGGL((msm_radix_scatter_kernel<512, 8, true, false, false>), grid, dim3(512), 0, st, a);
            else if (first) hipLaunchKernelGGL((msm_radix_scatter_kernel<1024, 8, true, false, false>), grid, dim3(1024), 0, st, a);
            else if (last && a.pk_in_bits) hipLaunchKernelGGL((msm_radix_scatter_kernel<512, 8, false, true, true>), grid, dim3(512), 0, st, a);
            else if (last) hipLaunchKernelGGL((msm_radix_scatter_kernel<256, 16, false, true, false>), grid, dim3(256), 0, st, a);
            else hipLaunchKernelGGL((msm_radix_scatter_kernel<1024, 8, false, false, false>), grid, dim3(1024), 0, st, a);
        }
    }
    g.cnt_cur = m.lvl_cnt[0].as<uint32_t>();
    g.off_cur = m.lvl_off[0].as<uint32_t>();
    g.base_cur = sm + 1024;
    g.part_cur = m.lvl_part[0].as<XYZZ>();
    uint32_t* len_hist = sm + 3328;
    uint32_t* len_cur = sm + 3328 + kLenBins;
    g.direct = direct_ok;
    XYZZ* direct_buckets = g.direct ? m.buckets.as<XYZZ>() : nullptr;
    {
        KernelScope ks(c, "msm_scan_win");
        hipLaunchKernelGGL(msm_scan_win_kernel, dim3(g.Wd), dim3(1024), scan_win_lds(g.NB), st, bcount, g.L, g.cnt_cur, g.off_cur, win_tot,
                           d_max, g.NB, len_hist, g.cut);
        hipLaunchKernelGGL(msm_win_base_kernel, dim3(1), dim3(1024), 0, st, win_tot, g.base_cur, g.Wd);
    }
    TaskDesc* desc = m.task_desc.as<TaskDesc>();
    {
        KernelScope ks(c, "msm_task_order");
        uint32_t* big_count = sm + 3908;
        UZK_TRY(m.big.reserve((size_t)(g.TBK + 1) * sizeof(BigBucket)));
        hipLaunchKernelGGL(msm_task_scan_kernel, dim3(1), dim3(256), 0, st, len_hist, len_cur);
        hipLaunchKernelGGL(msm_bucket_fill_kernel, dim3((unsigned)((g.TBK + 255) / 256)), dim3(256), 0, st, g.base_cur, g.cnt_cur, g.off_cur,
                           bstart, bcount, g.NB, g.TBK, len_cur, desc, big_count, m.big.as<BigBucket>(), g.direct ? 1u : 0u, g.cut);
        hipLaunchKernelGGL(msm_task_fill_big_kernel, dim3(1024), dim3(64), 0, st, big_count, m.big.as<BigBucket>(), len_cur, desc);
    }
    {
        KernelScope ks(c, "msm_accumulate");
        const dim3 grid((unsigned)((g.bound0 + 255) / 256));
        uint32_t* exc_count = sm + 3900;
        uint32_t* exc_list = m.exc.as<uint32_t>();
        hipLaunchKernelGGL(msm_accumulate29_kernel, grid, dim3(256), 0, st, points, sorted, desc, g.base_cur, g.part_cur,
                           g.Wd, exc_count, exc_list, direct_buckets);
        hipLaunchKernelGGL(msm_accumulate_exc_kernel, dim3(std::min<unsigned>(grid.x, 128u)), dim3(256), 0, st, points, sorted, desc, g.part_cur,
                           exc_count, exc_list, direct_buckets);
    }
    UZK_HIP(hipGetLastError());
    UZK_HIP(hipMemcpyAsync(m.h_max, d_max, 8, hipMemcpyDeviceToHost, st));
    return UZK_OK;
}

static int msm_group_phase2(Ctx& c, MsmGroup& g, bool accumulate = false, bool reduce = true) {
    const int a29 = (c.tune_arith29 >> 2) & 1;
    MsmWork& m = *g.m;
    hipStream_t st = g.st;
    c.cur_stream = st;
    UZK_HIP(hipStreamSynchronize(st));
    uint32_t* sm = m.small.as<uint32_t>();
    uint32_t* win_tot = sm;
    uint32_t* win_base[2] = {sm + 1024, sm + 2080};
    XYZZ* buckets = m.buckets.as<XYZZ>();
    XYZZ* partials = m.partials.as<XYZZ>();
    XYZZ* win_sums = m.win_sums.as<XYZZ>();
    const uint32_t G = kCombineFan;
    static_assert(kCutMaxTasks <= kCombineFan, "a short-cut bucket must never need a fold level of its own");
    uint64_t tmax = m.h_max[1];
    const uint32_t gs = g.TBK >= (1u << 18) ? 1u : (tmax > 2 ? 4u : 1u);
    constexpr uint32_t kBigThresh = 4;
    static_assert(sizeof(BigFold) == sizeof(BigBucket), "the two lists share one buffer");
    const bool big_mode = gs == 1 && tmax > kBigThresh;
    uint32_t* big_count = sm + 3904;
    BigFold* big_list = nullptr;
    if (big_mode) {
        UZK_TRY(m.big.reserve((size_t)(g.bound0 / G + g.TBK + 1) * sizeof(BigFold)));
        big_list = m.big.as<BigFold>();
    }
    if (g.direct && tmax > G) {
        KernelScope ks(c, "msm_combine");
        hipLaunchKernelGGL(msm_undirect_kernel, dim3((unsigned)((g.TBK + 255) / 256)), dim3(256), 0, st, buckets, g.cnt_cur, g.off_cur,
                           g.base_cur, g.part_cur, g.NB, g.TBK);
        g.direct = false;
    }
    if (accumulate && g.direct) { set_error("msm: direct bucket writes in an accumulating chunk (internal error)"); return UZK_ERR_DEVICE; }
    const int skip_single = g.direct ? 1 : 0;
    int lvl = 0;
    uint64_t bound_prev = g.bound0;
    const MsmCut fin_cut = tmax > G ? MsmCut() : g.cut;
    while (tmax > G) {
        const int nx = (lvl + 1) & 1;
        UZK_TRY(m.lvl_part[nx].reserve((size_t)g.part_cap * sizeof(XYZZ)));
        uint32_t* cnt_nx = m.lvl_cnt[nx].as<uint32_t>();
        uint32_t* off_nx = m.lvl_off[nx].as<uint32_t>();
        uint32_t* base_nx = win_base[nx];
        const uint64_t bound_nx = bound_prev / G + g.TBK;
        XYZZ* part_nx = m.lvl_part[nx].as<XYZZ>();
        {
            KernelScope ks(c, "msm_scan_win");
            hipLaunchKernelGGL(msm_scan_win_kernel, dim3(g.Wd), dim3(1024), scan_win_lds(g.NB), st, g.cnt_cur, G, cnt_nx, off_nx, win_tot,
                               (uint32_t*)nullptr, g.NB);
            hipLaunchKernelGGL(msm_win_base_kernel, dim3(1), dim3(1024), 0, st, win_tot, base_nx, g.Wd);
        }
        {
            KernelScope ks(c, "msm_combine");
            const dim3 grid((unsigned)((bound_nx * gs + 255) / 256));
            if (gs == 16)
                hipLaunchKernelGGL(msm_combine_kernel<16>, grid, dim3(256), 0, st, g.part_cur, g.cnt_cur, g.off_cur, g.base_cur,
                                   off_nx, base_nx, part_nx, g.NB, g.Wd, G, (uint32_t*)nullptr, (BigFold*)nullptr, 0u, a29);
            else if (gs == 4)
                hipLaunchKernelGGL(msm_combine_kernel<4>, grid, dim3(256), 0, st, g.part_cur, g.cnt_cur, g.off_cur, g.base_cur,
                                   off_nx, base_nx, part_nx, g.NB, g.Wd, G, (uint32_t*)nullptr, (BigFold*)nullptr, 0u, a29);
            else {
                if (big_mode) UZK_HIP(hipMemsetAsync(big_count, 0, 4, st));
                hipLaunchKernelGGL(msm_combine_kernel<1>, grid, dim3(256), 0, st, g.part_cur, g.cnt_cur, g.off_cur, g.base_cur,
                                   off_nx, base_nx, part_nx, g.NB, g.Wd, G, big_count, big_list, kBigThresh, a29);
                if (big_mode)
                    hipLaunchKernelGGL(msm_fold_big_kernel, dim3(2048), dim3(64), 0, st, g.part_cur, big_count, big_list, part_nx, 0);
            }
        }
        g.cnt_cur = cnt_nx; g.off_cur = off_nx; g.base_cur = base_nx; g.part_cur = part_nx;
        bound_prev = bound_nx;
        tmax = (tmax + G - 1) / G;
        lvl = nx;
    }
    {
        KernelScope ks(c, "msm_finalize");
        const dim3 grid((unsigned)((g.TBK * gs + 255) / 256));
        if (gs == 16)
            hipLaunchKernelGGL(msm_finalize_kernel<16>, grid, dim3(256), 0, st, g.part_cur, g.cnt_cur, g.off_cur, g.base_cur,
                               buckets, g.NB, g.Wd, accumulate ? 1 : 0, (uint32_t*)nullptr, (BigFold*)nullptr, 0u, skip_single, a29, fin_cut);
        else if (gs == 4)
            hipLaunchKernelGGL(msm_finalize_kernel<4>, grid, dim3(256), 0, st, g.part_cur, g.cnt_cur, g.off_cur, g.base_cur,
                               buckets, g.NB, g.Wd, accumulate ? 1 : 0, (uint32_t*)nullptr, (BigFold*)nullptr, 0u, skip_single, a29, fin_cut);
        else {
            const bool big_last = big_mode && tmax > kBigThresh;
            if (big_last) UZK_HIP(hipMemsetAsync(big_count, 0, 4, st));
            hipLaunchKernelGGL(msm_finalize_kernel<1>, grid, dim3(256), 0, st, g.part_cur, g.cnt_cur, g.off_cur, g.base_cur,
                               buckets, g.NB, g.Wd, accumulate ? 1 : 0, big_count, big_last ? big_list : (BigFold*)nullptr, kBigThresh, skip_single, a29, fin_cut);
            if (big_last)
                hipLaunchKernelGGL(msm_fold_big_kernel, dim3(2048), dim3(64), 0, st, g.part_cur, big_count, big_list, buckets, accumulate ? 1 : 0);
        }
    }
    if (!reduce) { UZK_HIP(hipGetLastError()); return UZK_OK; }
    if (g.class_s) {
        XYZZ* cls = m.class_sums.as<XYZZ>();
        const uint32_t RW2 = g.RW * 2;
        {
            KernelScope ks(c, "msm_reduce_class");
            hipLaunchKernelGGL(msm_class_sums_kernel, dim3(g.NBL / 2048, g.RW, 2), dim3(256), 0, st, buckets, cls, g.NBL, g.class_s, g.nb2, (c.tune_arith29 >> 2) & 1);
        }
        {
            KernelScope ks(c, "msm_reduce");
            const uint32_t seg2 = 4, log_seg2 = 2, groups2 = (g.nb2 + seg2 * kQuadLanes - 1) / (seg2 * kQuadLanes);
            XYZZ* part_r = partials + (size_t)RW2 * groups2;
            hipLaunchKernelGGL(msm_reduce_scan_quad_kernel, dim3(groups2, RW2), dim3(kQuadLanes * 4), 0, st, cls, groups2 == 1 ? win_sums : partials,
                               part_r, g.nb2, groups2, seg2, log_seg2);
            if (groups2 > 1)
                hipLaunchKernelGGL(msm_fold_scan_quad_kernel, dim3(RW2), dim3(kQuadLanes * 4), 0, st, partials, part_r, win_sums, groups2,
                                   kLogQuadLanes + log_seg2);
        }
        UZK_HIP(hipGetLastError());
        UZK_HIP(hipMemcpyAsync(m.h_sums, win_sums, (size_t)RW2 * sizeof(XYZZ), hipMemcpyDeviceToHost, st));
        return UZK_OK;
    }
    {
        KernelScope ks(c, "msm_reduce");
        if (g.scan_reduce) {
            XYZZ* part_r = partials + (size_t)g.RW * g.groups;
            uint32_t log_seg = 0;
            while ((1u << log_seg) < g.seg) ++log_seg;
            if (g.quad_reduce) {
                hipLaunchKernelGGL(msm_reduce_scan_quad_kernel, dim3(g.groups, g.RW), dim3(kQuadLanes * 4), 0, st, buckets, partials, part_r,
                                   g.NBL, g.groups, g.seg, log_seg);
                hipLaunchKernelGGL(msm_fold_scan_quad_kernel, dim3(g.RW), dim3(kQuadLanes * 4), 0, st, partials, part_r, win_sums, g.groups,
                                   kLogQuadLanes + log_seg);
            } else {
                hipLaunchKernelGGL(msm_reduce_scan_kernel, dim3(g.groups, g.RW), dim3(256), 0, st, buckets, partials, part_r, g.NBL,
                                   g.groups, g.seg, log_seg);
                hipLaunchKernelGGL(msm_fold_scan_kernel, dim3(g.RW), dim3(256), 0, st, partials, part_r, win_sums, g.groups,
                                   8 + log_seg);
            }
        } else {
            hipLaunchKernelGGL(msm_reduce_kernel, dim3(g.groups, g.RW), dim3(256), 0, st, buckets, partials, g.NBL, g.groups, g.seg);
            hipLaunchKernelGGL(msm_fold_partials_kernel, dim3(g.RW), dim3(256), 0, st, partials, win_sums, g.groups);
        }
    }
    UZK_HIP(hipGetLastError());
    UZK_HIP(hipMemcpyAsync(m.h_sums, win_sums, (size_t)g.RW * sizeof(XYZZ), hipMemcpyDeviceToHost, st));
    return UZK_OK;
}

namespace {
class HornerPool {
public:
    explicit HornerPool(unsigned nthreads) {
        for (unsigned t = 0; t < nthreads; ++t) workers_.emplace_back([this] { loop(); });
    }
    ~HornerPool() {
        { std::lock_guard<std::mutex> lk(mu_); stop_ = true; }
        cv_.notify_all();
        for (auto& w : workers_) w.join();
    }
    void run(uint32_t count, const std::function<void(uint32_t)>& fn) {
        auto job = std::make_shared<Job>();
        job->fn = &fn;
        job->count = count;
        { std::lock_guard<std::mutex> lk(mu_); active_.push_back(job); }
        cv_.notify_all();
        work(*job);
        std::unique_lock<std::mutex> lk(mu_);
        cv_done_.wait(lk, [&] { return job->done.load() >= count; });
        for (size_t i = 0; i < active_.size(); ++i)
            if (active_[i] == job) { active_.erase(active_.begin() + (long)i); break; }
    }
private:
    struct Job {
        const std::function<void(uint32_t)>* fn = nullptr;
        uint32_t count = 0;
        std::atomic<uint32_t> next{0}, done{0};
    };
    void work(Job& j) {
        for (;;) {
            const uint32_t i = j.next.fetch_add(1);
            if (i >= j.count) break;
            (*j.fn)(i);
            if (j.done.fetch_add(1) + 1 >= j.count) { std::lock_guard<std::mutex> lk(mu_); cv_done_.notify_all(); }
        }
    }
    std::shared_ptr<Job> pending_locked() const {
        for (const auto& j : active_) if (j->next.load() < j->count) return j;
        return nullptr;
    }
    void loop() {
        for (;;) {
            std::shared_ptr<Job> j;
            {
                std::unique_lock<std::mutex> lk(mu_);
                cv_.wait(lk, [&] { return stop_ || (j = pending_locked()) != nullptr; });
                if (stop_) return;
            }
            work(*j);
        }
    }
    std::vector<std::thread> workers_;
    std::mutex mu_;
    std::condition_variable cv_, cv_done_;
    std::vector<std::shared_ptr<Job>> active_;
    bool stop_ = false;
};
HornerPool& horner_pool() {
    static HornerPool pool(7);
    return pool;
}
}

template <class WindowSum>
static void msm_horner_host(Ctx& c, uint32_t batch, uint32_t wpp, int cb, const WindowSum& window_sum, Jac* out_host, int class_s = 0) {
    auto horner = [&](uint32_t b) {
        if (class_s > 0)
            out_host[b] = h64::horner_split(wpp, std::max(cb, class_s), class_s, [&](uint32_t w) -> const XYZZ& { return (&window_sum(b, w))[0]; },
                                            [&](uint32_t w) -> const XYZZ& { return (&window_sum(b, w))[1]; });
        else
            out_host[b] = h64::horner(wpp, cb, [&](uint32_t w) -> const XYZZ& { return window_sum(b, w); });
    };
    HostScope hs_horner(c, "host_msm_horner");
    if (batch > 1 && wpp > 1) {
        const std::function<void(uint32_t)> job = [&](uint32_t b) { horner(b); };
        horner_pool().run(batch, job);
    } else {
        for (uint32_t b = 0; b < batch; ++b) horner(b);
    }
}

static int small_window_bits(Ctx& c, size_t n, uint32_t batch) {
    if (c.msm_window_bits >= 4 && c.msm_window_bits <= 10) return c.msm_window_bits;
    (void)batch;
    if (n <= 256) return 5;
    if (n <= 2048) return 7;
    return 8;
}
bool msm_small_applies(Ctx& c, size_t n, uint32_t batch, int pre_c = 0) {
    if (!c.tune_small || n == 0 || n > (1u << 15)) return false;
    if (pre_c > 10 || (pre_c == 0 && c.msm_window_bits > 10)) return false;
    const int cb = pre_c > 0 ? pre_c : small_window_bits(c, n, batch);
    const uint64_t S = (uint64_t)batch * (uint64_t)msm_num_windows(cb);
    return S <= 65535 && S * n < (1ull << 31);
}

static int msm_run_small(Ctx& c, const Affine* points, const ScalarView& d_scalars, size_t n, uint32_t batch, Jac* out_host, int pre_c,
                         uint32_t pre_stride, uint32_t pre_off) {
    MsmWork& m = c.msm[0];
    hipStream_t st = c.stream;
    c.cur_stream = st;
    const int cb = pre_c > 0 ? pre_c : small_window_bits(c, n, batch);
    const uint32_t W = (uint32_t)msm_num_windows(cb), S = batch * W, NBL = 1u << (cb - 1), n32 = (uint32_t)n;
    const uint64_t entries = (uint64_t)S * n;
    uint32_t L = 0;
    {
        const double lanes = 0.93 * 64.0 * 4.0 * (double)c.num_cus;
        for (int k = 1; k <= 4; ++k) {
            L = (uint32_t)((double)entries / (lanes * k)) + 1;
            if (L <= 12) break;
        }
        L = std::max<uint32_t>(L, 2);
    }
    const uint64_t task_cap = entries / L + (uint64_t)S * NBL;
    SmallLevels lv{};
    uint64_t cap[kSmallMaxLevels + 1];
    cap[0] = task_cap;
    {
        uint64_t worst = (n + L - 1) / L;
        while (worst > 1 && lv.nl < (uint32_t)kSmallMaxLevels) { worst = (worst + kSmallFan - 1) / kSmallFan; ++lv.nl; }
        if (worst > 1) { set_error("msm: small pipeline: %u fold levels do not cover n = %zu at task length %u", lv.nl, n, L); return UZK_ERR_PARAMETER; }
    }
    uint64_t p_total = 0, d_total = 0;
    for (uint32_t k = 0; k <= lv.nl; ++k) {
        if (k > 0) cap[k] = cap[k - 1] / kSmallFan + (uint64_t)S * NBL;
        lv.pbase[k] = (uint32_t)p_total;
        lv.dbase[k] = (uint32_t)d_total;
        p_total += cap[k];
        if (k > 0) d_total += cap[k];
    }
    if (p_total >= (1ull << 32)) { set_error("msm: small pipeline: too many partial sums"); return UZK_ERR_PARAMETER; }
    UZK_TRY(m.digits.reserve((size_t)entries * 4));
    UZK_TRY(m.sorted.reserve((size_t)entries * 4));
    UZK_TRY(m.task_desc.reserve((size_t)task_cap * sizeof(TaskDesc)));
    UZK_TRY(m.lvl_part[0].reserve((size_t)p_total * sizeof(XYZZ)));
    UZK_TRY(m.exc.reserve((size_t)task_cap * 4));
    UZK_TRY(m.partials.reserve((size_t)(d_total + 1) * sizeof(SmallChunk)));
    UZK_TRY(m.bucket_count.reserve((size_t)S * NBL * 4));
    UZK_TRY(m.bucket_start.reserve((size_t)S * kSmallMaxLevels * sizeof(uint2)));
    UZK_TRY(m.win_sums.reserve((size_t)S * sizeof(XYZZ)));
    UZK_TRY(m.small.reserve(16384));
    if (m.h_sums_cap < S) {
        if (m.h_sums) (void)hipHostFree(m.h_sums);
        UZK_HIP(hipHostMalloc(reinterpret_cast<void**>(&m.h_sums), (size_t)S * sizeof(XYZZ), hipHostMallocDefault));
        m.h_sums_cap = S;
    }
    uint32_t* digits = m.digits.as<uint32_t>();
    uint32_t* sorted = m.sorted.as<uint32_t>();
    TaskDesc* desc = m.task_desc.as<TaskDesc>();
    XYZZ* P = m.lvl_part[0].as<XYZZ>();
// ... 200 lines not shown
```

Baseline: 873.1 million points/s.

## Add speculative MSM phase-2 launch, split radix scan totals, and compact segment list

Adds an opt-in speculative phase-2 path that queues finalize and reduce kernels without first syncing to read the max bucket occupancy. Each kernel checks a device-side gate and exits early if the occupancy exceeds the assumed limit, in which case the host reruns the normal path. The first-pass radix scan now computes per-group totals in a separate kernel, so later groups no longer rescan all earlier rows. Later passes take a compacted list of active segments built in the items kernel instead of launching one block per segment, and packed-key entry buffers are sized smaller. The speculative path is off by default, so the default run only sees the sort-scan restructuring.

```diff
diff --git a/uzkge_amd/csrc/api.cpp b/uzkge_amd/csrc/api.cpp
--- a/uzkge_amd/csrc/api.cpp
+++ b/uzkge_amd/csrc/api.cpp
@@ -330,7 +330,7 @@
     to.tune_no_precompute = from.tune_no_precompute; to.tune_ntt_tile = from.tune_ntt_tile; to.tune_ntt_two_pass = from.tune_ntt_two_pass; to.tune_small = from.tune_small;
     to.tune_chunk_log = from.tune_chunk_log; to.tune_verify_transcript = from.tune_verify_transcript; to.tune_stream_log = from.tune_stream_log; to.tune_stream_min_log = from.tune_stream_min_log;
     to.tune_seg_sort = from.tune_seg_sort; to.tune_arith29 = from.tune_arith29;
-    to.tune_msm_taper = from.tune_msm_taper;
+    to.tune_msm_taper = from.tune_msm_taper; to.tune_sort_grid = from.tune_sort_grid; to.tune_msm_spec = from.tune_msm_spec;
 }
 }
 int uzk_ctx_create(uint64_t* ctx_out) try {
@@ -1989,6 +1989,8 @@
     else if (!std::strcmp(key, "msm_small")) c.tune_small = value ? 1 : 0;
     else if (!std::strcmp(key, "msm_seg_sort")) c.tune_seg_sort = value;
     else if (!std::strcmp(key, "msm_taper")) c.tune_msm_taper = (value >= 0 && value <= 2) ? value : 1;
+    else if (!std::strcmp(key, "msm_sort_grid")) c.tune_sort_grid = (value >= 0 && value <= 65535) ? value : 0;
+    else if (!std::strcmp(key, "msm_spec")) c.tune_msm_spec = value ? 1 : 0;
     else if (!std::strcmp(key, "ntt_tile")) c.tune_ntt_tile = (value == 1024 || value == 2048) ? value : 0;
     else if (!std::strcmp(key, "ntt_two_pass")) c.tune_ntt_two_pass = value ? 1 : 0;
     else if (!std::strcmp(key, "arith29")) c.tune_arith29 = value & 7;
diff --git a/uzkge_amd/csrc/ctx.hpp b/uzkge_amd/csrc/ctx.hpp
--- a/uzkge_amd/csrc/ctx.hpp
+++ b/uzkge_amd/csrc/ctx.hpp
@@ -103,6 +103,8 @@
     }
     int tune_seg_sort = 1;
     int tune_msm_taper = 1;
+    int tune_sort_grid = 0;
+    int tune_msm_spec = 0;
     DevBuf poly_tmp, poly_tmp2, poly_io, zpoly_tmp, open_tmp, poly_args;
     DevBuf poly_cnt;
     uint32_t trim_flip = 0;
diff --git a/uzkge_amd/csrc/msm.hip b/uzkge_amd/csrc/msm.hip
--- a/uzkge_amd/csrc/msm.hip
+++ b/uzkge_amd/csrc/msm.hip
@@ -224,57 +224,85 @@
 }
 
 __global__ __launch_bounds__(512) void msm_radix_scan_kernel(RadixArgs a, uint32_t nch, const uint32_t* __restrict__ out_start_of,
-                                                             uint32_t out_stride) {
+                                                             uint32_t out_stride, const uint32_t* __restrict__ group_tot,
+                                                             const uint32_t* __restrict__ seg_list) {
     __shared__ uint32_t wsum[8];
+    const uint32_t b = threadIdx.x, G = gridDim.y, g = blockIdx.y;
+    const uint32_t todo = seg_list ? seg_list[0] : gridDim.x;
+    for (uint32_t it = blockIdx.x; it < todo; it += gridDim.x) {
+        const uint32_t seg = seg_list ? seg_list[1 + it] : it;
+        uint32_t run = 0;
+        if (b < a.bins) {
+            size_t first = (size_t)seg * nch;
+            uint32_t cnt = nch;
+            if (a.item_off) { first = a.item_off[seg]; cnt = a.item_off[seg + 1] - a.item_off[seg]; }
+            const uint32_t per = (cnt + G - 1) / G;
+            const uint32_t c0 = min(cnt, g * per), c1 = min(cnt, c0 + per);
+            const uint32_t* p0 = group_tot ? group_tot + (size_t)seg * G * a.bins + b : a.counts + first * a.bins + b;
+            const uint32_t rows = group_tot ? g : c0;
+            uint32_t r0 = 0, r1 = 0, r2 = 0, r3 = 0;
+            uint32_t ch = 0;
+            for (; ch + 4 <= rows; ch += 4) {
+                r0 += p0[(size_t)ch * a.bins];
+                r1 += p0[(size_t)(ch + 1) * a.bins];
+                r2 += p0[(size_t)(ch + 2) * a.bins];
+                r3 += p0[(size_t)(ch + 3) * a.bins];
+            }
+            for (; ch < rows; ++ch) r0 += p0[(size_t)ch * a.bins];
+            run = r0 + r1 + r2 + r3;
+            for (ch = c0; ch < c1; ++ch) {
+                const size_t at = (first + ch) * a.bins + b;
+                const uint32_t v = a.counts[at];
+                a.prefix[at] = run;
+                run += v;
+            }
+        }
+        if (g + 1 != G) return;
+        uint32_t incl = run;
+        for (int o = 1; o < 64; o <<= 1) {
+            const uint32_t t = __shfl_up((int)incl, o);
+            if ((int)(b & 63) >= o) incl += t;
+        }
+        if ((b & 63) == 63) wsum[b >> 6] = incl;
+        __syncthreads();
+        uint32_t pre = 0;
+        for (uint32_t w = 0; w < (b >> 6); ++w) pre += wsum[w];
+        const uint32_t excl = pre + incl - run;
+        if (b < a.bins) {
+            const uint32_t start = out_start_of ? out_start_of[seg] : seg * out_stride;
+            a.bin_base[(size_t)seg * a.bins + b] = start + excl;
+            a.bin_count[(size_t)seg * a.bins + b] = run;
+        }
+        __syncthreads();
+    }
+}
+
+__global__ __launch_bounds__(512) void msm_radix_group_totals_kernel(const uint32_t* __restrict__ counts, uint32_t nch, uint32_t bins,
+                                                                     uint32_t* __restrict__ group_tot) {
     const uint32_t seg = blockIdx.x, b = threadIdx.x, G = gridDim.y, g = blockIdx.y;
-    if (a.seg_min_len && a.seg_len[seg] <= a.seg_min_len) return;
-    uint32_t run = 0;
-    if (b < a.bins) {
-        size_t first = (size_t)seg * nch;
-        uint32_t cnt = nch;
-        if (a.item_off) { first = a.item_off[seg]; cnt = a.item_off[seg + 1] - a.item_off[seg]; }
-        const uint32_t per = (cnt + G - 1) / G;
-        const uint32_t c0 = min(cnt, g * per), c1 = min(cnt, c0 + per);
-        const uint32_t* p0 = a.counts + first * a.bins + b;
-        uint32_t r0 = 0, r1 = 0, r2 = 0, r3 = 0;
-        uint32_t ch = 0;
-        for (; ch + 4 <= c0; ch += 4) {
-            r0 += p0[(size_t)ch * a.bins];
-            r1 += p0[(size_t)(ch + 1) * a.bins];
-            r2 += p0[(size_t)(ch + 2) * a.bins];
-            r3 += p0[(size_t)(ch + 3) * a.bins];
-        }
-        for (; ch < c0; ++ch) r0 += p0[(size_t)ch * a.bins];
-        run = r0 + r1 + r2 + r3;
-        for (ch = c0; ch < c1; ++ch) {
-            const size_t at = (first + ch) * a.bins + b;
-            const uint32_t v = a.counts[at];
-            a.prefix[at] = run;
-            run += v;
-        }
-    }
-    if (g + 1 != G) return;
-    uint32_t incl = run;
-    for (int o = 1; o < 64; o <<= 1) {
-        const uint32_t t = __shfl_up((int)incl, o);
-        if ((int)(b & 63) >= o) incl += t;
-    }
-    if ((b & 63) == 63) wsum[b >> 6] = incl;
-    __syncthreads();
-    uint32_t pre = 0;
-    for (uint32_t w = 0; w < (b >> 6); ++w) pre += wsum[w];
-    const uint32_t excl = pre + incl - run;
-    if (b < a.bins) {
-        const uint32_t start = out_start_of ? out_start_of[seg] : seg * out_stride;
-        a.bin_base[(size_t)seg * a.bins + b] = start + excl;
-        a.bin_count[(size_t)seg * a.bins + b] = run;
-    }
+    if (b >= bins) return;
+    const uint32_t per = (nch + G - 1) / G;
+    const uint32_t c0 = min(nch, g * per), c1 = min(nch, c0 + per);
+    const uint32_t* p0 = counts + (size_t)seg * nch * bins + b;
+    uint32_t r0 = 0, r1 = 0, r2 = 0, r3 = 0;
+    uint32_t ch = c0;
+    for (; ch + 4 <= c1; ch += 4) {
+        r0 += p0[(size_t)ch * bins];
+        r1 += p0[(size_t)(ch + 1) * bins];
+        r2 += p0[(size_t)(ch + 2) * bins];
+        r3 += p0[(size_t)(ch + 3) * bins];
+    }
+    for (; ch < c1; ++ch) r0 += p0[(size_t)ch * bins];
+    group_tot[((size_t)seg * G + g) * bins + b] = r0 + r1 + r2 + r3;
 }
 
 __global__ __launch_bounds__(1024) void msm_radix_items_kernel(const uint32_t* __restrict__ seg_len, uint32_t nseg,
-                                                               uint32_t chunk, uint32_t* __restrict__ item_off, uint32_t min_len) {
+                                                               uint32_t chunk, uint32_t* __restrict__ item_off, uint32_t min_len,
+                                                               uint32_t* __restrict__ seg_list) {
     __shared__ uint32_t part[1024];
+    __shared__ uint32_t listed;
     const uint32_t tid = threadIdx.x;
+    if (tid == 0) listed = 0;
     const uint32_t per = (nseg + 1023) / 1024;
     const uint32_t lo = min(nseg, tid * per), hi = min(nseg, lo + per);
     uint32_t s = 0;
@@ -289,8 +317,14 @@
         __syncthreads();
     }
     uint32_t run = part[tid] - s;
-    for (uint32_t k = lo; k < hi; ++k) { item_off[k] = run; run += items_of(k); }
+    for (uint32_t k = lo; k < hi; ++k) {
+        item_off[k] = run;
+        run += items_of(k);
+        if (min_len == 0 || seg_len[k] > min_len) seg_list[1 + atomicAdd(&listed, 1u)] = k;
+    }
     if (tid == 1023) item_off[nseg] = part[1023];
+    __syncthreads();
+    if (tid == 0) seg_list[0] = listed;
 }
 
 template <int TB, int E, bool FROM_DIGITS, bool OUT_VAL, bool PK_IN>
@@ -862,13 +896,17 @@
     }
 }
 
+struct SpecGate { const uint32_t* max; uint32_t lim; };
+__device__ __forceinline__ bool spec_lost(const SpecGate& gate) { return gate.max != nullptr && gate.max[1] > gate.lim; }
+
 template <int GS>
 __global__ __launch_bounds__(256) void msm_finalize_kernel(const XYZZ* __restrict__ in, const uint32_t* __restrict__ in_cnt,
                                                            const uint32_t* __restrict__ in_off,
                                                            const uint32_t* __restrict__ in_base,
                                                            XYZZ* __restrict__ buckets, uint32_t NB, uint32_t W, int accumulate,
                                                            uint32_t* __restrict__ big_count, BigFold* __restrict__ big, uint32_t big_thresh,
-                                                           int skip_single, int arith29, MsmCut cut = MsmCut()) {
+                                                           int skip_single, int arith29, MsmCut cut, SpecGate gate) {
+    if (spec_lost(gate)) return;
     const size_t gt = (size_t)blockIdx.x * blockDim.x + threadIdx.x;
     size_t t = gt / GS;
     const uint32_t sub = (uint32_t)(gt % GS);
@@ -899,8 +937,9 @@
 }
 
 __global__ __launch_bounds__(256) void msm_reduce_kernel(const XYZZ* __restrict__ buckets, XYZZ* __restrict__ partials,
-                                                         uint32_t nbk, uint32_t groups_per_window, uint32_t seg) {
+                                                         uint32_t nbk, uint32_t groups_per_window, uint32_t seg, SpecGate gate) {
     __shared__ XYZZ sh[256];
+    if (spec_lost(gate)) return;
     const uint32_t w = blockIdx.y, tid = threadIdx.x;
     const uint32_t g = blockIdx.x * blockDim.x + tid;
     const XYZZ* bw = buckets + (size_t)w * nbk;
@@ -937,8 +976,9 @@
     if (tid == 0) partials[(size_t)w * groups_per_window + blockIdx.x] = sh[0];
 }
 __global__ __launch_bounds__(256) void msm_fold_partials_kernel(const XYZZ* __restrict__ partials, XYZZ* __restrict__ out,
-                                                                uint32_t groups) {
+                                                                uint32_t groups, SpecGate gate) {
     __shared__ XYZZ sh[256];
+    if (spec_lost(gate)) return;
     const uint32_t w = blockIdx.x, tid = threadIdx.x;
     XYZZ acc = xyzz_inf();
     for (uint32_t g = tid; g < groups; g += 256) { XYZZ q = partials[(size_t)w * groups + g]; xyzz_add(acc, q); }
@@ -982,8 +1022,9 @@
 }
 __global__ __launch_bounds__(256) void msm_reduce_scan_kernel(const XYZZ* __restrict__ buckets, XYZZ* __restrict__ part_p1,
                                                               XYZZ* __restrict__ part_r, uint32_t nbk,
-                                                              uint32_t groups_per_window, uint32_t seg, uint32_t log_seg) {
+                                                              uint32_t groups_per_window, uint32_t seg, uint32_t log_seg, SpecGate gate) {
     __shared__ XYZZ sh[256];
+    if (spec_lost(gate)) return;
     const uint32_t w = blockIdx.y, tid = threadIdx.x;
     const uint32_t g = blockIdx.x * blockDim.x + tid;
     const XYZZ* bw = buckets + (size_t)w * nbk;
@@ -1017,8 +1058,9 @@
     }
 }
 __global__ __launch_bounds__(256) void msm_fold_scan_kernel(const XYZZ* __restrict__ part_p1, const XYZZ* __restrict__ part_r,
-                                                            XYZZ* __restrict__ out, uint32_t groups, uint32_t log_shift) {
+                                                            XYZZ* __restrict__ out, uint32_t groups, uint32_t log_shift, SpecGate gate) {
     __shared__ XYZZ sh[256];
+    if (spec_lost(gate)) return;
     const uint32_t w = blockIdx.x, tid = threadIdx.x;
     XYZZ r = tid < groups ? part_r[(size_t)w * groups + tid] : xyzz_inf();
     XYZZ p1 = tid < groups ? part_p1[(size_t)w * groups + tid] : xyzz_inf();
@@ -1038,8 +1080,9 @@
 }
 
 __global__ __launch_bounds__(256, 3) void msm_class_sums_kernel(const XYZZ* __restrict__ buckets, XYZZ* __restrict__ out, uint32_t nbk,
-                                                              uint32_t log_s, uint32_t nb2, int arith29) {
+                                                              uint32_t log_s, uint32_t nb2, int arith29, SpecGate gate) {
     __shared__ XYZZ sh[256];
+    if (spec_lost(gate)) return;
     const uint32_t tile = blockIdx.x, w = blockIdx.y, cols = blockIdx.z, t = threadIdx.x;
     const uint32_t Lc = 1u << log_s, H = nbk >> log_s;
     const XYZZ* bw = buckets + (size_t)w * nbk;
@@ -1118,8 +1161,9 @@
 }
 __global__ __launch_bounds__(kQuadLanes * 4) void msm_reduce_scan_quad_kernel(const XYZZ* __restrict__ buckets, XYZZ* __restrict__ part_p1,
                                                                     XYZZ* __restrict__ part_r, uint32_t nbk,
-                                                                    uint32_t groups_per_window, uint32_t seg, uint32_t log_seg) {
+                                                                    uint32_t groups_per_window, uint32_t seg, uint32_t log_seg, SpecGate gate) {
     __shared__ XYZZ sh[kQuadLanes];
+    if (spec_lost(gate)) return;
     const uint32_t w = blockIdx.y, t = threadIdx.x >> 2, q = threadIdx.x & 3;
     const uint32_t g = blockIdx.x * kQuadLanes + t;
     const XYZZ* bw = buckets + (size_t)w * nbk;
@@ -1153,8 +1197,9 @@
     }
 }
 __global__ __launch_bounds__(kQuadLanes * 4) void msm_fold_scan_quad_kernel(const XYZZ* __restrict__ part_p1, const XYZZ* __restrict__ part_r,
-                                                                  XYZZ* __restrict__ out, uint32_t groups, uint32_t log_shift) {
+                                                                  XYZZ* __restrict__ out, uint32_t groups, uint32_t log_shift, SpecGate gate) {
     __shared__ XYZZ sh[kQuadLanes];
+    if (spec_lost(gate)) return;
     const uint32_t w = blockIdx.x, t = threadIdx.x >> 2, q = threadIdx.x & 3;
     XYZZ r = t < groups ? part_r[(size_t)w * groups + t] : xyzz_inf();
     XYZZ p1 = t < groups ? part_p1[(size_t)w * groups + t] : xyzz_inf();
@@ -1672,7 +1717,8 @@
     return UZK_OK;
 }
 
-struct SortPass { uint32_t shift, bins, nseg, nch, chunk, items_bound; };
+struct SortPass { uint32_t shift, bins, nseg, nch, chunk, items_bound, scan_g; };
+constexpr uint32_t kSortTailGrid = 2048, kSortTailScanGrid = 256;
 constexpr int kSegCfgs = 6;
 constexpr uint32_t kSegCap[kSegCfgs] = {128 * 12, 256 * 12, 256 * 24, 256 * 40, 512 * 40, 512 * 72};
 
@@ -1763,6 +1809,7 @@
         if (p == 0 && g.pk_bits && avg <= (1ull << 25)) g.sp[p].nch = (uint32_t)((avg + 32767) / 32768);
         g.sp[p].chunk = (p == g.P - 1) ? 16384u : 32768u;
         g.sp[p].items_bound = (uint32_t)(g.entries / g.sp[p].chunk) + nseg;
+        g.sp[p].scan_g = p == 0 ? std::max<uint32_t>(1, std::min<uint32_t>(g.sp[p].nch / 16, 1024 / std::max<uint32_t>(1, nseg))) : 1u;
         nseg *= g.sp[p].bins;
     }
     MsmWork& m = *g.m;
@@ -1775,12 +1822,12 @@
     UZK_TRY(m.win_sums.reserve((size_t)g.RW * 2 * sizeof(XYZZ)));
     if (g.class_s) UZK_TRY(m.class_sums.reserve((size_t)g.RW * 2 * g.nb2 * sizeof(XYZZ)));
     for (int p = 0; p < g.P; ++p) {
-        UZK_TRY(m.counts[p].reserve((size_t)(p == 0 ? 2 * g.sp[p].nseg * g.sp[p].nch : g.sp[p].items_bound) * g.sp[p].bins * 4));
-        if (p > 0) UZK_TRY(m.items[p].reserve(((size_t)g.sp[p].nseg + 1) * 4));
+        UZK_TRY(m.counts[p].reserve((p == 0 ? (size_t)g.sp[p].nseg * (2 * (size_t)g.sp[p].nch + g.sp[p].scan_g) : (size_t)g.sp[p].items_bound) * g.sp[p].bins * 4));
+        if (p > 0) UZK_TRY(m.items[p].reserve((2 * (size_t)g.sp[p].nseg + 2) * 4));
         if (p + 1 < g.P) {
             UZK_TRY(m.segs_start[p].reserve((size_t)g.sp[p].nseg * g.sp[p].bins * 4));
             UZK_TRY(m.segs_len[p].reserve((size_t)g.sp[p].nseg * g.sp[p].bins * 4));
-            UZK_TRY(m.ent[p & 1].reserve((size_t)g.entries * sizeof(uint2)));
+            UZK_TRY(m.ent[p & 1].reserve((size_t)g.entries * (g.pk_bits ? 4 : sizeof(uint2))));
         }
     }
     for (int k = 0; k < 2; ++k) {
@@ -1862,18 +1909,20 @@
             a.chunk = sp.chunk;
             KernelScope ks(c, "msm_sort_items");
             hipLaunchKernelGGL(msm_radix_items_kernel, dim3(1), dim3(1024), 0, st, a.seg_len, a.nseg, a.chunk,
-                               m.items[p].as<uint32_t>(), a.seg_min_len);
-        }
-        const dim3 grid = first ? dim3(sp.nch, sp.nseg) : dim3(seg_cfg >= 0 ? std::min<uint32_t>(sp.items_bound, 2048u) : sp.items_bound);
+                               m.items[p].as<uint32_t>(), a.seg_min_len, m.items[p].as<uint32_t>() + sp.nseg + 1);
+        }
+        const uint32_t tail_cap = c.tune_sort_grid > 0 ? (uint32_t)c.tune_sort_grid : (seg_cfg >= 0 ? kSortTailGrid : sp.items_bound);
+        const uint32_t scan_cap = c.tune_sort_grid > 0 ? (uint32_t)c.tune_sort_grid : (seg_cfg >= 0 ? kSortTailScanGrid : sp.nseg);
+        const dim3 grid = first ? dim3(sp.nch, sp.nseg) : dim3(std::min<uint32_t>(sp.items_bound, tail_cap));
         {
-            const size_t wgs = first ? 2 * (size_t)grid.x * grid.y : (size_t)sp.items_bound;
+            const size_t wgs = first ? (size_t)grid.y * (2 * (size_t)grid.x + sp.scan_g) : (size_t)sp.items_bound;
             const size_t ent_bytes = g.pk_bits ? 4 : sizeof(uint2);
             const bool ok = m.counts[p].cap >= wgs * sp.bins * 4 &&
                             (last ? (m.bucket_start.cap >= (size_t)sp.nseg * sp.bins * 4 && m.bucket_count.cap >= (size_t)sp.nseg * sp.bins * 4 &&
                                      m.sorted.cap >= (size_t)g.entries * 4)
                                   : (m.segs_start[p].cap >= (size_t)sp.nseg * sp.bins * 4 && m.segs_len[p].cap >= (size_t)sp.nseg * sp.bins * 4 &&
                                      m.ent[p & 1].cap >= (size_t)g.entries * ent_bytes)) &&
-                            (first || m.items[p].cap >= ((size_t)sp.nseg + 1) * 4);
+                            (first || m.items[p].cap >= (2 * (size_t)sp.nseg + 2) * 4);
             if (!ok) { set_error("msm: sort pass %d: a workspace is smaller than its launch needs (internal error)", p); return UZK_ERR_DEVICE; }
         }
         if (seg_cfg >= 0) {
@@ -1896,9 +1945,16 @@
         }
         {
             KernelScope ks(c, "msm_sort_scan");
-            const uint32_t scan_g = first ? std::max<uint32_t>(1, std::min<uint32_t>(sp.nch / 16, 1024 / std::max<uint32_t>(1, sp.nseg))) : 1u;
-            hipLaunchKernelGGL(msm_radix_scan_kernel, dim3(sp.nseg, scan_g), dim3(512), 0, st, a, sp.nch,
-                               first ? (const uint32_t*)nullptr : a.seg_start, first ? g.seg_n : 0u);
+            if (first) {
+                uint32_t* group_tot = sp.scan_g > 1 ? a.counts + 2 * (size_t)sp.nseg * sp.nch * sp.bins : nullptr;
+                if (group_tot)
+                    hipLaunchKernelGGL(msm_radix_group_totals_kernel, dim3(sp.nseg, sp.scan_g), dim3(512), 0, st, a.counts, sp.nch, sp.bins, group_tot);
+                hipLaunchKernelGGL(msm_radix_scan_kernel, dim3(sp.nseg, sp.scan_g), dim3(512), 0, st, a, sp.nch, (const uint32_t*)nullptr,
+                                   g.seg_n, group_tot, (const uint32_t*)nullptr);
+            } else {
+                hipLaunchKernelGGL(msm_radix_scan_kernel, dim3(std::min<uint32_t>(sp.nseg, scan_cap)), dim3(512), 0, st, a, sp.nch, a.seg_start,
+                                   0u, (const uint32_t*)nullptr, m.items[p].as<uint32_t>() + sp.nseg + 1);
+            }
         }
         {
             KernelScope ks(c, "msm_sort_scatter");
@@ -1953,13 +2009,17 @@
     return UZK_OK;
 }
 
-static int msm_group_phase2(Ctx& c, MsmGroup& g, bool accumulate = false, bool reduce = true) {
+constexpr uint32_t kBigThresh = 4;
+static uint32_t msm_spec_limit(const MsmGroup& g) { return g.TBK >= (1u << 18) ? kBigThresh : 2u; }
+
+static int msm_group_phase2_queue(Ctx& c, MsmGroup& g, bool accumulate, bool reduce, bool spec) {
     const int a29 = (c.tune_arith29 >> 2) & 1;
     MsmWork& m = *g.m;
     hipStream_t st = g.st;
     c.cur_stream = st;
-    UZK_HIP(hipStreamSynchronize(st));
+    if (!spec) UZK_HIP(hipStreamSynchronize(st));
     uint32_t* sm = m.small.as<uint32_t>();
+    const SpecGate gate{spec ? sm + 3200 : nullptr, msm_spec_limit(g)};
     uint32_t* win_tot = sm;
     uint32_t* win_base[2] = {sm + 1024, sm + 2080};
     XYZZ* buckets = m.buckets.as<XYZZ>();
@@ -1967,9 +2027,8 @@
     XYZZ* win_sums = m.win_sums.as<XYZZ>();
     const uint32_t G = kCombineFan;
     static_assert(kCutMaxTasks <= kCombineFan, "a short-cut bucket must never need a fold level of its own");
-    uint64_t tmax = m.h_max[1];
+    uint64_t tmax = spec ? msm_spec_limit(g) : m.h_max[1];
     const uint32_t gs = g.TBK >= (1u << 18) ? 1u : (tmax > 2 ? 4u : 1u);
-    constexpr uint32_t kBigThresh = 4;
     static_assert(sizeof(BigFold) == sizeof(BigBucket), "the two lists share one buffer");
     const bool big_mode = gs == 1 && tmax > kBigThresh;
     uint32_t* big_count = sm + 3904;
@@ -2030,15 +2089,15 @@
         const dim3 grid((unsigned)((g.TBK * gs + 255) / 256));
         if (gs == 16)
             hipLaunchKernelGGL(msm_finalize_kernel<16>, grid, dim3(256), 0, st, g.part_cur, g.cnt_cur, g.off_cur, g.base_cur,
-                               buckets, g.NB, g.Wd, accumulate ? 1 : 0, (uint32_t*)nullptr, (BigFold*)nullptr, 0u, skip_single, a29, fin_cut);
+                               buckets, g.NB, g.Wd, accumulate ? 1 : 0, (uint32_t*)nullptr, (BigFold*)nullptr, 0u, skip_single, a29, fin_cut, gate);
         else if (gs == 4)
             hipLaunchKernelGGL(msm_finalize_kernel<4>, grid, dim3(256), 0, st, g.part_cur, g.cnt_cur, g.off_cur, g.base_cur,
-                               buckets, g.NB, g.Wd, accumulate ? 1 : 0, (uint32_t*)nullptr, (BigFold*)nullptr, 0u, skip_single, a29, fin_cut);
+                               buckets, g.NB, g.Wd, accumulate ? 1 : 0, (uint32_t*)nullptr, (BigFold*)nullptr, 0u, skip_single, a29, fin_cut, gate);
         else {
             const bool big_last = big_mode && tmax > kBigThresh;
             if (big_last) UZK_HIP(hipMemsetAsync(big_count, 0, 4, st));
             hipLaunchKernelGGL(msm_finalize_kernel<1>, grid, dim3(256), 0, st, g.part_cur, g.cnt_cur, g.off_cur, g.base_cur,
-                               buckets, g.NB, g.Wd, accumulate ? 1 : 0, big_count, big_last ? big_list : (BigFold*)nullptr, kBigThresh, skip_single, a29, fin_cut);
+                               buckets, g.NB, g.Wd, accumulate ? 1 : 0, big_count, big_last ? big_list : (BigFold*)nullptr, kBigThresh, skip_single, a29, fin_cut, gate);
             if (big_last)
                 hipLaunchKernelGGL(msm_fold_big_kernel, dim3(2048), dim3(64), 0, st, g.part_cur, big_count, big_list, buckets, accumulate ? 1 : 0);
         }
@@ -2049,17 +2108,17 @@
         const uint32_t RW2 = g.RW * 2;
         {
             KernelScope ks(c, "msm_reduce_class");
-            hipLaunchKernelGGL(msm_class_sums_kernel, dim3(g.NBL / 2048, g.RW, 2), dim3(256), 0, st, buckets, cls, g.NBL, g.class_s, g.nb2, (c.tune_arith29 >> 2) & 1);
+            hipLaunchKernelGGL(msm_class_sums_kernel, dim3(g.NBL / 2048, g.RW, 2), dim3(256), 0, st, buckets, cls, g.NBL, g.class_s, g.nb2, (c.tune_arith29 >> 2) & 1, gate);
         }
         {
             KernelScope ks(c, "msm_reduce");
             const uint32_t seg2 = 4, log_seg2 = 2, groups2 = (g.nb2 + seg2 * kQuadLanes - 1) / (seg2 * kQuadLanes);
             XYZZ* part_r = partials + (size_t)RW2 * groups2;
             hipLaunchKernelGGL(msm_reduce_scan_quad_kernel, dim3(groups2, RW2), dim3(kQuadLanes * 4), 0, st, cls, groups2 == 1 ? win_sums : partials,
-                               part_r, g.nb2, groups2, seg2, log_seg2);
+                               part_r, g.nb2, groups2, seg2, log_seg2, gate);
             if (groups2 > 1)
                 hipLaunchKernelGGL(msm_fold_scan_quad_kernel, dim3(RW2), dim3(kQuadLanes * 4), 0, st, partials, part_r, win_sums, groups2,
-                                   kLogQuadLanes + log_seg2);
+                                   kLogQuadLanes + log_seg2, gate);
         }
         UZK_HIP(hipGetLastError());
         UZK_HIP(hipMemcpyAsync(m.h_sums, win_sums, (size_t)RW2 * sizeof(XYZZ), hipMemcpyDeviceToHost, st));
@@ -2073,23 +2132,32 @@
             while ((1u << log_seg) < g.seg) ++log_seg;
             if (g.quad_reduce) {
                 hipLaunchKernelGGL(msm_reduce_scan_quad_kernel, dim3(g.groups, g.RW), dim3(kQuadLanes * 4), 0, st, buckets, partials, part_r,
-                                   g.NBL, g.groups, g.seg, log_seg);
+                                   g.NBL, g.groups, g.seg, log_seg, gate);
                 hipLaunchKernelGGL(msm_fold_scan_quad_kernel, dim3(g.RW), dim3(kQuadLanes * 4), 0, st, partials, part_r, win_sums, g.groups,
-                                   kLogQuadLanes + log_seg);
+                                   kLogQuadLanes + log_seg, gate);
             } else {
                 hipLaunchKernelGGL(msm_reduce_scan_kernel, dim3(g.groups, g.RW), dim3(256), 0, st, buckets, partials, part_r, g.NBL,
-                                   g.groups, g.seg, log_seg);
+                                   g.groups, g.seg, log_seg, gate);
                 hipLaunchKernelGGL(msm_fold_scan_kernel, dim3(g.RW), dim3(256), 0, st, partials, part_r, win_sums, g.groups,
-                                   8 + log_seg);
+                                   8 + log_seg, gate);
             }
         } else {
-            hipLaunchKernelGGL(msm_reduce_kernel, dim3(g.groups, g.RW), dim3(256), 0, st, buckets, partials, g.NBL, g.groups, g.seg);
-            hipLaunchKernelGGL(msm_fold_partials_kernel, dim3(g.RW), dim3(256), 0, st, partials, win_sums, g.groups);
+            hipLaunchKernelGGL(msm_reduce_kernel, dim3(g.groups, g.RW), dim3(256), 0, st, buckets, partials, g.NBL, g.groups, g.seg, gate);
+            hipLaunchKernelGGL(msm_fold_partials_kernel, dim3(g.RW), dim3(256), 0, st, partials, win_sums, g.groups, gate);
         }
     }
     UZK_HIP(hipGetLastError());
     UZK_HIP(hipMemcpyAsync(m.h_sums, win_sums, (size_t)g.RW * sizeof(XYZZ), hipMemcpyDeviceToHost, st));
     return UZK_OK;
+}
+
+static int msm_group_phase2(Ctx& c, MsmGroup& g, bool accumulate = false, bool reduce = true) {
+    if (c.tune_msm_spec) {
+        UZK_TRY(msm_group_phase2_queue(c, g, accumulate, reduce,  true));
+        UZK_HIP(hipStreamSynchronize(g.st));
+        if (g.m->h_max[1] <= msm_spec_limit(g)) return UZK_OK;
+    }
+    return msm_group_phase2_queue(c, g, accumulate, reduce,  false);
 }
 
 namespace {
```

Result: no change. 872.8 million points/s (-0.0%).
